# tyb311/TCCT

Measured on AMD Instinct MI355X. Metric: OCT B-scans/sec fwd+bwd(+clip+AdamW), stc_tt bs=8 1x800x1100, higher is better.
Workload: dtype bf16; 1 GPU; stc_tt --los=di bs=8/GPU 1x800x1100 (net tensors 3x800x1104); global_batch=8, parallelism=dp1, ranks=1, grad_allreduce=none, slowest_step=115

## Files before the change

include/tcct_hip.h:

```cpp
#ifndef TCCT_HIP_H
#define TCCT_HIP_H
#include <stdint.h>
#ifdef __cplusplus
extern "C" {
#endif

typedef void* tcct_stream_t;

enum { TCCT_F32 = 0, TCCT_BF16 = 1 };
enum { TCCT_ACT_NONE = 0, TCCT_ACT_LRELU = 1, TCCT_ACT_HSWISH = 2, TCCT_ACT_GELU = 3, TCCT_ACT_SIGMOID = 4,
       TCCT_ACT_ABS = 5 };
enum { TCCT_CRIT_DICE = 0, TCCT_CRIT_DICE2 = 1, TCCT_CRIT_IOU = 2, TCCT_CRIT_MSE = 3 };
enum { TCCT_MCRIT_DICE = 0, TCCT_MCRIT_DICE2 = 1, TCCT_MCRIT_IOU = 2, TCCT_MCRIT_CE = 3 };

int tcct_version(void);
const char* tcct_last_error(void);
int tcct_set_outputs_prezeroed(int on);

int tcct_image_to_nhwc4(const float* img, void* out, int N, int Csrc, int H, int Wsrc, int Wdst, int dtype,
                        tcct_stream_t stream);
int tcct_u8_gather2d(const uint8_t* src, uint8_t* dst, int N, int SH, int SW, int C, int sy0, int sx0, int sh, int sw, int DH, int DW,
                     int dy0, int dx0, int dh, int dw, int flipy, int flipx, int mul, int div, int fill, tcct_stream_t stream);
int tcct_onehot_to_index(const int64_t* onehot, uint8_t* lab, int N, int C, int64_t HW, tcct_stream_t stream);
int tcct_labels_to_u8(const int64_t* lab, uint8_t* out, int N, int H, int Wsrc, int Wdst, tcct_stream_t stream);
// ... 85 lines not shown
                       tcct_stream_t stream);
int tcct_conv32f_pack_weights_sub(const float* w, float* wp, int KH, int KW, int transposed, int cin_total, int o_off, int i_off, tcct_stream_t stream);
int tcct_conv32f_fwd_strided(const float* x, const float* wp, const float* bias, float* y, int N, int H, int W, int KH, int KW, int PH, int PW, int xs,
                             int xo, int ys, int yo, int accumulate, tcct_stream_t stream);
int tcct_conv32f_wgrad_strided(const float* x, const float* dy, float* dw, float* dbias, int N, int H, int W, int KH, int KW, int PH, int PW, int xs,
                               int xo, int ds, int dof, int ldi, int o_off, int i_off, tcct_stream_t stream);
int tcct_pwf_fwd(const float* x, const float* w, const float* bias, float* y, int64_t M, int K, int N, int transposed, tcct_stream_t stream);
int tcct_pwf_wgrad(const float* x, const float* dy, float* dw, float* dbias, int64_t M, int K, int N, tcct_stream_t stream);
int tcct_conv32_pack_weights(const float* w, void* wp, int KH, int KW, int transposed, tcct_stream_t stream);
int tcct_conv32_pack_weights_multi(const void* desc, int n, tcct_stream_t stream);
int tcct_conv32_pack_weights_both(const float* w, void* wp2, int KH, int KW, tcct_stream_t stream);
int tcct_conv32_fwd(const void* x, const void* wp, const float* bias, void* y, int N, int H, int W, int KH, int KW, int PH,
                    int PW, tcct_stream_t stream);

int tcct_conv32_fwd_bnstats(const void* x, const void* wp, const float* bias, void* y, int N, int H, int W, int KH, int KW, int PH,
                            int PW, double* stats, int pre_act, tcct_stream_t stream);
int tcct_conv32_fwd_affine(const void* x, const void* wp, const float* bias, void* y, int N, int H, int W, int KH, int KW,
                           int PH, int PW, const float* ab, int pre_act, int post_act, tcct_stream_t stream);
int tcct_pw_fwd_affine(const void* x, const float* w, const float* bias, void* y, int64_t M, int K, int N, const float* ab,
                       int pre_act, int post_act, int out_dtype, tcct_stream_t stream);
int tcct_pw_fwd_affine_residual(const void* x, const float* w, const float* bias, const float* ab, const void* res, void* y, int64_t M, int K, int N,
                                tcct_stream_t stream);
int tcct_pw_fwd_cat2_affine(const void* x1, const void* x2, const float* w, const float* bias, const float* ab, int post_act, void* y, int64_t M, int K, int N,
                            tcct_stream_t stream);
int tcct_pw_fwd_xaff_affine_residual(const void* y_prev, const float* ab_prev, const float* w, const float* bias, const float* ab, const void* res, void* y,
                                     int64_t M, int K, int N, tcct_stream_t stream);
int tcct_conv32_fwd_add(const void* x, const void* wp, const float* bias, const void* res, void* y, int N, int H, int W, int KH, int KW,
                        int PH, int PW, tcct_stream_t stream);
int tcct_conv32_chain33(const void* x, const void* wp1, const float* bias1, void* mid, const void* wp2, const float* bias2, void* y,
                        const void* res, int N, int H, int W, double* stats, tcct_stream_t stream);
int tcct_conv32_pack_weights_sub(const float* w, void* wp, int KH, int KW, int transposed, int cin_total, int o_off, int i_off,
                                 tcct_stream_t stream);
int tcct_conv32_fwd_strided(const void* x, const void* wp, const float* bias, void* y, int N, int H, int W, int KH, int KW, int PH,
                            int PW, int xs, int xo, int ys, int yo, int accumulate, tcct_stream_t stream);
int tcct_conv32_fwd_strided_bnstats(const void* x, const void* wp, const float* bias, void* y, int N, int H, int W, int KH, int KW, int PH,
                                    int PW, int xs, int xo, int ys, int yo, int accumulate, double* stats, int pre_act, tcct_stream_t stream);
int tcct_conv32_fwd_strided_affine(const void* x, const void* wp, const float* bias, void* y, int N, int H, int W, int KH, int KW, int PH, int PW, int xs,
                                   int xo, int ys, int yo, const float* ab, int pre_act, int post_act, tcct_stream_t stream);
int64_t tcct_conv32_wgrad_mode(int mode);
int64_t tcct_conv32_fwd_mode(int mode);
int tcct_conv32_wgrad_strided(const void* x, const void* dy, float* dw, float* dbias, int N, int H, int W, int KH, int KW, int PH,
                              int PW, int xs, int xo, int ds, int dof, int cin_total, int o_off, int i_off, tcct_stream_t stream);
int tcct_conv32x64_fwd33(const void* x, const void* wp, int wps, const float* bias, void* y, int N, int H, int W, double* stats, int pre_act, int force,
                         tcct_stream_t stream);
int tcct_conv32x64_wgrad33(const void* x, const void* dy, float* dw, float* dbias, int N, int H, int W, int force, tcct_stream_t stream);
int tcct_conv64x32_dgrad33(const void* dy, const void* wp_t, int wps, void* dx, int N, int H, int W, int force, tcct_stream_t stream);
int tcct_conv32_wgrad(const void* x, const void* dy, float* dw, float* dbias, int N, int H, int W, int KH, int KW, int PH,
                      int PW, tcct_stream_t stream);
int tcct_conv32_bwd3x3(const void* x, const void* dy, const void* wp_t, const void* dskip, void* dx, float* dw, float* dbias, int N, int H,
                       int W, tcct_stream_t stream);

int tcct_pw_fwd(const void* x, const float* w, const float* bias, void* y, int64_t M, int K, int N, int transposed,
                int out_dtype, tcct_stream_t stream);
int tcct_pw_wgrad(const void* x, const void* dy, float* dw, float* dbias, int64_t M, int K, int N, tcct_stream_t stream);
int tcct_pw_bwd(const void* x, const void* dy, const float* w, const void* res, void* dx, float* dw, float* dbias, int64_t M, int K, int N,
                tcct_stream_t stream);
int tcct_pw_bwd_cat2(const void* x1, const void* x2, const void* dy, const float* w, void* dx1, void* dx2, float* dw, int64_t M, int K, int N,
                     tcct_stream_t stream);
int tcct_pw_bwd_residual2(const void* x, const void* dy, const float* w, const void* res, void* dx_sum, void* dx_plain, float* dw, float* dbias,
                          int64_t M, int K, int N, tcct_stream_t stream);
int64_t tcct_pw_bwd_bn_supported(int K, int N, int post, int red_post, int split);
int tcct_pw_bwd_bn(const void* x, const void* x2, const void* dz, const void* y, const float* coef, int post, const float* w, const void* res,
                   void* dx, void* dx2, float* dw, float* dbias, int64_t M, int K, int N, const void* y_prev, const float* ab_prev,
                   int red_post, double* sums_prev, tcct_stream_t stream);
int tcct_pw_bwd_bn_sums(const void* x, const void* x2, const void* dz, const void* y, const double* sums, int raw, const float* mean_rstd,
                        const float* ab, float* dgamma, float* dbeta, int post, const float* w, const void* res, void* dx, void* dx2, float* dw,
                        float* dbias, int64_t M, int K, int N, const void* y_prev, const float* ab_prev, int red_post, double* sums_prev,
                        tcct_stream_t stream);
int tcct_pw_wgrad_strided(const void* x, const void* dy, int64_t ldy, float* dw, float* dbias, int64_t M, int K, int N,
                          tcct_stream_t stream);
int tcct_pw_fwd_residual(const void* x, const float* w, const float* bias, const void* res, const float* scale, int64_t per_sample,
                         void* y, void* y_plain, int64_t M, int K, int N, tcct_stream_t stream);
int tcct_pw_fwd_bnstats_xaff(const void* y_prev, const float* ab_prev, const float* w, const float* bias, void* y, int64_t M, int K, int N, double* stats,
                             tcct_stream_t stream);
int tcct_pw_bwd_bn_sums_xaff(const void* y_prev, const float* ab_prev, const void* dz, const void* y, const double* sums, int raw, const float* mean_rstd,
                             const float* ab, float* dgamma, float* dbeta, const float* w, const void* res, void* dx, float* dw, float* dbias, int64_t M,
                             int K, int N, int red_post, double* sums_prev, tcct_stream_t stream);
int tcct_pw_fwd_gelu_residual(const void* x1, const float* w, const float* bias, const void* res, const float* scale, int64_t per_sample, void* y,
                              int64_t M, int K, int N, tcct_stream_t stream);
int tcct_pw_bwd_residual2_sum(const void* x, const void* dy_a, const void* dy_b, const float* w, const void* res, void* dx_sum, void* dx_plain, float* dw,
                              float* dbias, int64_t M, int K, int N, tcct_stream_t stream);
int tcct_pw_bwd_lnb(const void* x, const void* dy, const float* w, const void* t, const float* mean_rstd, const float* gamma, const void* res, void* dt,
                    float* dw, float* dbias, float* dgamma, float* dbeta, int64_t M, int K, int N, tcct_stream_t stream);
int tcct_pw_bwd_gelu(const void* x1, const void* dy, const float* w, void* dx1, float* dw, float* dbias, int64_t M, int K, int N, tcct_stream_t stream);
int tcct_pw_dgrad_residual(const void* dy, const float* w, const void* res, void* dx_sum, void* dx_plain, int64_t M, int Nout, int K,
                           tcct_stream_t stream);
int tcct_pw_fwd_cat2(const void* x1, const void* x2, int K1, const float* w, const float* bias, void* y, int64_t M, int K, int N,
                     double* stats, int pre_act, tcct_stream_t stream);
int tcct_pw_fwd_f32_upadd(const void* x, const float* w, const float* bias, float* y, int B, int uH, int uW, int K, int N, const float* up, tcct_stream_t stream);
int tcct_pw_dgrad_split2(const void* dy, const float* w, void* dx1, void* dx2, int K1, int64_t M, int Nout, int K, tcct_stream_t stream);
int tcct_pw_bwd_cat2_bias(const void* x1, const void* x2, const void* dy, const float* w, void* dx1, void* dx2, float* dw, float* dbias, int64_t M,
                          int K, int N, tcct_stream_t stream);
int tcct_tail_compose(const float* w1, const float* b1, const float* w2, const float* b2, float* wc, float* c, tcct_stream_t stream);
int tcct_tail_compose_bwd(const float* w1, const float* b1, const float* w2, const float* dwc, const float* dc, float* dw1, float* db1, float* dw2,
                          float* db2, tcct_stream_t stream);
int tcct_tail_compose3(const float* w1, const float* b1, const float* w2, const float* b2, const float* w3, const float* b3, int C, float* wcc, float* wa,
                       float* wb, float* ccc, tcct_stream_t stream);
int tcct_tail_compose3_bwd(const float* w1, const float* b1, const float* w2, const float* b2, const float* w3, int C, const float* dwa, const float* dwb,
                           const float* dccc, float* dw1, float* db1, float* dw2, float* db2, float* dw3, float* db3, tcct_stream_t stream);
int tcct_pw_fwd_cat2_f32(const void* x1, const void* x2, int K1, const float* w, const float* bias, float* y, int64_t M, int K, int N, tcct_stream_t stream);
int tcct_head_compose(const float* wt, const float* bt, const float* wa, const float* ba, int C, float* wh, float* ch, tcct_stream_t stream);
int tcct_head_compose_bwd(const float* wt, const float* bt, const float* wa, int C, const float* dwh, const float* dch, float* dwt, float* dbt,
                          float* dwa, float* dba, tcct_stream_t stream);
int tcct_pw_wgrad_cat2(const void* x1, const void* x2, int K1, const void* dy, float* dw, float* dbias, int64_t M, int K, int N,
                       tcct_stream_t stream);
int tcct_pw_fwd_bnstats(const void* x, const float* w, const float* bias, void* y, int64_t M, int K, int N, double* stats, int pre_act,
                        tcct_stream_t stream);

int tcct_im2col3x3_c3(const void* x4, void* out, int N, int H, int W, int stride, int dtype, tcct_stream_t stream);
int tcct_c3_fwd(const void* x4, const float* w, const float* bias, void* y, int B, int H, int W, int stride, double* stats, int stat_pre,
                const float* ab, int pre_act, int post_act, tcct_stream_t stream);
int tcct_c3_wgrad(const void* x4, const void* dy, float* dw, float* dbias, int B, int H, int W, int stride, tcct_stream_t stream);
int tcct_c3_bn_fwd_train(const void* x4, const float* w, const float* bias, void* z, int B, int H, int W, int stride, double* sums,
                         const float* gamma, const float* beta, float eps, float momentum, float* running_mean, float* running_var,
                         int64_t* num_batches_tracked, float* mean_rstd, float* ab, int post_act, tcct_stream_t stream);
int tcct_c3_bn_fwd_eval(const void* x4, const float* w, const float* bias, void* z, int B, int H, int W, int stride, const float* ab, int post_act,
                        tcct_stream_t stream);
int tcct_c3_bn_bwd_reduce(const void* x4, const float* w, const float* bias, const void* dz, int B, int H, int W, int stride, const float* ab,
                          double* raw, int post_act, tcct_stream_t stream);
int tcct_c3_bn_bwd_wgrad(const void* x4, const float* w, const float* bias, const void* dz, int B, int H, int W, int stride, const float* coef,
                         float* dw, float* dbias, int post_act, tcct_stream_t stream);
int64_t tcct_c3_bn_bwd_prefetch(int tiles_ahead);
int tcct_c3_bn_bwd_onepass(const void* x4, const float* w, const float* bias, const void* dz, int B, int H, int W, int stride, const float* mean_rstd,
                           const float* ab, float* work, double* sums, float* dw, float* dbias, float* dgamma, float* dbeta, int post_act, tcct_stream_t stream);
int tcct_pw_wgrad_smalln(const void* x, const void* dy, float* dw, float* dbias, int64_t M, int K, int N, int x_dtype,
                         int dy_dtype, tcct_stream_t stream);

int tcct_stream_copy(const void* src, void* dst, int64_t nbytes, tcct_stream_t stream);

int64_t tcct_kernel_census(int which, int reset);
int tcct_marker(int id, tcct_stream_t stream);

int tcct_dwconv3x3_fwd(const void* x, const float* w, const float* bias, void* y, int N, int H, int W, int C,
                       int stride, int add_input, int dtype, tcct_stream_t stream);
int tcct_dwconv3x3_fwd_bnstats(const void* x, const float* w, const float* bias, void* y, int N, int H, int W, int C, int stride,
                               int add_input, double* stats, int dtype, tcct_stream_t stream);
int tcct_dwconv3x3_dgrad(const void* dy, const float* w, void* dx, int N, int H, int W, int C, int stride,
                         int add_input, int dtype, tcct_stream_t stream);
int tcct_dwconv3x3_dgrad_add(const void* dy, const float* w, const void* res, void* dx, int N, int H, int W, int C, int stride,
                             int add_input, int dtype, tcct_stream_t stream);
int tcct_dwconv3x3_wgrad(const void* x, const void* dy, float* dw, float* dbias, int N, int H, int W, int C,
                         int stride, int dtype, tcct_stream_t stream);
int tcct_dwconv3x3_fwd_xaff(const void* x, const float* xab, const float* w, const float* bias, void* y, int N, int H, int W, int C, int stride,
                            double* stats, int dtype, tcct_stream_t stream);
int tcct_dwconv3x3_wgrad_xaff(const void* x, const float* xab, const void* dy, float* dw, float* dbias, int N, int H, int W, int C, int stride, int dtype,
                              tcct_stream_t stream);
int tcct_dwconv3x3_dgrad_bnred(const void* dy, const float* w, const void* y_prev, const float* ab_prev, void* dx, double* raw, int N, int H, int W, int C,
                               int dtype, tcct_stream_t stream);

int tcct_metapool_fwd(const void* x, void* y, int B, int64_t N, int C, int dtype, tcct_stream_t stream);
int tcct_metapool_bwd(const void* dy, void* dx, int B, int64_t N, int C, int dtype, tcct_stream_t stream);
int tcct_metapool_residual_fwd(const void* x, const void* res, const float* scale, void* y, int B, int64_t N, int C, int dtype,
                               tcct_stream_t stream);
int tcct_metapool_scaled_bwd(const void* dy, const float* scale, void* dx, int B, int64_t N, int C, int dtype, tcct_stream_t stream);
int tcct_ln_metapool_residual_fwd(const void* t, void* y, int B, int64_t N, int C, const float* gamma, const float* beta, float eps, const float* scale,
                                  int dtype, tcct_stream_t stream);
int tcct_ln_metapool_residual_ln_fwd(const void* t, void* y, void* y2, int B, int64_t N, int C, const float* gamma, const float* beta, float eps,
                                     const float* scale, const float* gamma2, const float* beta2, float eps2, float* mean_rstd2, int dtype, tcct_stream_t stream);
int tcct_ln_metapool_residual_bwd(const void* t, const void* dy, void* dt, int B, int64_t N, int C, const float* gamma, float eps, const float* scale,
                                  float* dgamma, float* dbeta, int dtype, tcct_stream_t stream);
int tcct_maxpool2_fwd(const void* x, void* y, int N, int H, int W, int C, int dtype, tcct_stream_t stream);
int tcct_maxpool2_bwd(const void* x, const void* dy, void* dx, int N, int H, int W, int C, int dtype, tcct_stream_t stream);
int tcct_maxpool2_bwd_add(const void* x, const void* dy, const void* res, void* dx, int N, int H, int W, int C, int dtype,
                          tcct_stream_t stream);
int tcct_bilinear_fwd(const void* x, void* y, int N, int H, int W, int C, int Ho, int Wo, int align_corners, int dtype,
                      tcct_stream_t stream);
int tcct_bilinear_bwd_separable(const float* dy, float* dx, float* workspace, int N, int H, int W, int C, int Ho, int Wo,
                                int align_corners, tcct_stream_t stream);
int tcct_bilinear_add_fwd(const void* x, const void* res, void* y, int N, int H, int W, int C, int Ho, int Wo, int align_corners,
                          int dtype, tcct_stream_t stream);
int64_t tcct_bilinear_bwd_x2(int on);
int tcct_bilinear_bwd(const void* dy, void* dx, int N, int H, int W, int C, int Ho, int Wo, int align_corners, int dtype,
                      tcct_stream_t stream);
int tcct_l2norm_fwd(const void* x, void* y, int64_t M, int C, float eps, int dtype, tcct_stream_t stream);
int tcct_l2norm_bwd(const void* x, const void* dy, void* dx, int64_t M, int C, float eps, int dtype, tcct_stream_t stream);
int tcct_l2norm_bwd_scaled(const void* x, const void* dy, void* dx, int64_t M, int C, float eps, float scale, int dtype,
                           tcct_stream_t stream);
int tcct_l2norm_bwd_scaled_add(const void* x, const void* dy, const void* res, void* dx, int64_t M, int C, float eps, float scale, int dtype,
                               tcct_stream_t stream);
int tcct_normadd_fwd(const void* g0, const void* g1, const void* g2, float* inv1, float* inv2, void* out, int N, int H, int W, int C,
                     int h1, int w1, int h2, int w2, float eps, int dtype, tcct_stream_t stream);
int tcct_normadd6_fwd(const void* a0, const void* b0, const void* a1, const void* b1, const void* a2, const void* b2, float* inv1, float* inv2,
                      void* out, int N, int H, int W, int C, int h1, int w1, int h2, int w2, float eps, int dtype, tcct_stream_t stream);
int tcct_l2norm_bwd2_scaled(const void* xa, const void* xb, const void* dn, const void* res_a, const void* res_b, void* da, void* db,
                            int64_t M, int C, float eps, float scale, int dtype, tcct_stream_t stream);

int tcct_softmax_dice_fwd(const void* logits, const uint8_t* labels, int64_t M, int C, double* sums, float* loss,
                          int dtype, tcct_stream_t stream);
int tcct_softmax_dice_bwd(const void* logits, const uint8_t* labels, int64_t M, int C, const double* sums,
                          const float* grad_out, float grad_scale, void* dlogits, int dtype, tcct_stream_t stream);
int tcct_updice_fwd(const float* low, const uint8_t* labels, int B, int h, int w, int H, int W, int C, double* sums, float* loss,
                    tcct_stream_t stream);
int tcct_updice_bwd(const float* low, const uint8_t* labels, int B, int h, int w, int H, int W, int C, const double* sums,
                    const float* grad_out, float grad_scale, float* ws, float* dlow, tcct_stream_t stream);
int tcct_dice_ds_fwd(const void* logits, int dtype, const uint8_t* labels, int B, int H, int W, int C, const float* low1, int h1, int w1, const float* low2,
                     int h2, int w2, const float* low3, int h3, int w3, float coff, double* sums, float* loss, tcct_stream_t stream);
int tcct_softmax_crit_fwd(const void* logits, const uint8_t* labels, int64_t M, int C, int kind, const float* class_w, double* sums, float* loss, int dtype,
                          tcct_stream_t stream);
int tcct_softmax_crit_bwd(const void* logits, const uint8_t* labels, int64_t M, int C, int kind, const float* class_w, const double* sums, const float* grad_out,
                          float grad_scale, void* dlogits, int dtype, tcct_stream_t stream);
int tcct_upcrit_fwd(const float* low, const uint8_t* labels, int B, int h, int w, int H, int W, int C, int kind, const float* class_w, double* sums, float* loss,
                    tcct_stream_t stream);
int tcct_upcrit_bwd(const float* low, const uint8_t* labels, int B, int h, int w, int H, int W, int C, int kind, const float* class_w, const double* sums,
                    const float* grad_out, float grad_scale, float* ws, float* dlow, tcct_stream_t stream);
int tcct_crit_ds_fwd(const void* logits, int dtype, const uint8_t* labels, int B, int H, int W, int C, const float* low1, int h1, int w1, const float* low2, int h2, int w2,
                     const float* low3, int h3, int w3, float coff, int kind, const float* class_w, double* sums, float* loss, tcct_stream_t stream);
int tcct_softmax_mcrit_fwd(const void* logits, const uint8_t* labels, int B, int64_t HW, int C, int kind, const float* class_w, double* sums, float* loss, int dtype,
                           tcct_stream_t stream);
int tcct_softmax_mcrit_bwd(const void* logits, const uint8_t* labels, int B, int64_t HW, int C, int kind, const float* class_w, const double* sums, const float* grad_out,
                           float grad_scale, void* dlogits, int dtype, tcct_stream_t stream);
int tcct_upmcrit_fwd(const float* low, const uint8_t* labels, int B, int h, int w, int H, int W, int C, int kind, const float* class_w, double* sums, float* loss,
                     tcct_stream_t stream);
int tcct_upmcrit_bwd(const float* low, const uint8_t* labels, int B, int h, int w, int H, int W, int C, int kind, const float* class_w, const double* sums,
                     const float* grad_out, float grad_scale, float* ws, float* dlow, tcct_stream_t stream);
int tcct_mcrit_ds_fwd(const void* logits, int dtype, const uint8_t* labels, int B, int H, int W, int C, const float* low1, int h1, int w1, const float* low2, int h2, int w2,
                      const float* low3, int h3, int w3, float coff, int kind, const float* class_w, double* sums, float* loss, tcct_stream_t stream);
int tcct_softmax_pick(const void* logits, const uint8_t* labels, int64_t M, int C, float* prob_lab, uint8_t* argmax,
                      int dtype, tcct_stream_t stream);
int tcct_confusion_counts(const uint8_t* pred, const uint8_t* labels, int N, int64_t HW, int C, float* out,
                          tcct_stream_t stream);

int tcct_gate_fusion_fwd(const void* x1, const void* x2, const float* field, void* y, int N, int H, int W, int C, int hs, int ws,
                         int dtype, tcct_stream_t stream);
int tcct_gate_fusion_bwd(const void* dy, const float* field, void* dx1, void* dx2, int N, int H, int W, int C, int hs, int ws,
                         int dtype, tcct_stream_t stream);

int tcct_mask_boundaries(const uint8_t* mask, int32_t* out, int N, int H, int W, int C, tcct_stream_t stream);

int tcct_slice_channels_fwd(const void* x, float* y, int64_t M, int C, int start, int n, int dtype, tcct_stream_t stream);
int tcct_slice_channels_bwd(const float* dy, void* dx, int64_t M, int C, int start, int n, int dtype, tcct_stream_t stream);
int tcct_label_planes(const uint8_t* labels, float* onehot, float* edge, int N, int H, int W, int start, int n,
                      tcct_stream_t stream);
int tcct_gumbel_colsoftmax_fwd(const float* x, const float* eps, float* out, float* stats, int N, int H, int W, int CH,
                               tcct_stream_t stream);
int tcct_gumbel_colsoftmax_bwd(const float* x, const float* eps, const float* stats, const float* dout, float* dx, int N,
                               int H, int W, int CH, tcct_stream_t stream);
int tcct_colsoftmax_fwd(const float* x, float* y, int N, int H, int W, tcct_stream_t stream);
int tcct_colsoftmax_bwd(const float* y, const float* dy, float* dx, int N, int H, int W, tcct_stream_t stream);
int tcct_colwsum_fwd(const float* x, const float* wts, float* out, int N, int H, int W, tcct_stream_t stream);
int tcct_colwsum_bwd(const float* dout, const float* wts, float* dx, int N, int H, int W, tcct_stream_t stream);
int tcct_mse_fwd(const float* a, const float* b, int64_t n, double* acc, float* out, tcct_stream_t stream);
// ... 55 lines not shown
```

tcct_amd/__init__.py:

```python
__version__ = '0.1.0'

import os as _os
import warnings as _warnings

RETIRED_ENV = frozenset('''TCCT_BILINEAR_VEC8 TCCT_BN_DEFER TCCT_BN_DEFER_DW TCCT_BN_FUSE TCCT_BN_POOL TCCT_BN_RED TCCT_BN_RED_DW TCCT_BN_VEC8 TCCT_C3_BN TCCT_C3_DIRECT
TCCT_C3_ONEPASS TCCT_CONV_STREAM TCCT_DP_MARKS TCCT_DS_DICE TCCT_DW_CPT TCCT_DW_WGRAD_CPT TCCT_DW_WGRAD_SIDE TCCT_DY2 TCCT_F32_MFMA TCCT_FPL_LAZY_GRAD
TCCT_FUSED_CONV_BWD TCCT_FUSED_PW_BWD TCCT_FUSE_AUX TCCT_GRAPH_ERRMODE TCCT_GRAPH_SHARED_POOL TCCT_HEAD_COMPOSE TCCT_HEAD_UPADD TCCT_LN_POOL TCCT_LN_POOL_LN2
TCCT_MLP_GELU TCCT_MLP_TAIL TCCT_NORMADD_BAND TCCT_PACK_ALL TCCT_PW_FWD2 TCCT_TAIL_AUX TCCT_TAIL_AUX_LOW TCCT_TAIL_COMPOSE TCCT_TRAN_FUSE TCCT_TRAN_RED2
TCCT_WGRAD_FRESH_EVENT TCCT_WGRAD_GENERIC TCCT_WGRAD_LINE TCCT_WGRAD_RECORD_STREAM TCCT_WGRAD_STREAM'''.split())
_set = sorted(v for v in RETIRED_ENV if v in _os.environ)
if _set:
    _warnings.warn('tcct_amd: ' + ', '.join(_set) + ' no longer have any effect (retired environment switches; use the tcct_amd.ops module constants or '
                   '`bench.py --set NAME=0|1`)', RuntimeWarning, stacklevel=2)
```

tcct_amd/csrc/common.h:

```cpp
#pragma once
#include <hip/hip_runtime.h>
#include <hip/hip_bf16.h>
#include <stdint.h>
#include <stdio.h>
#include "../../include/tcct_hip.h"

typedef __hip_bfloat16 bf16;

void tcct_set_error(const char* fmt, ...);
enum { TCCT_CENSUS_CHAIN33 = 0, TCCT_CENSUS_WGRADK_STREAM = 1, TCCT_CENSUS_WGRAD33_STREAM = 2, TCCT_CENSUS_FWD33_STREAM = 3, TCCT_CENSUS_N = 8 };
void tcct_census_hit(int which);
int tcct_skip_zero_fill();

#define TCCT_CHECK(cond, ...)                                   \
    do {                                                        \
        if (!(cond)) {                                          \
            tcct_set_error(__VA_ARGS__);                        \
            return -1;                                          \
        }                                                       \
    } while (0)

#define TCCT_LAUNCH_OK()                                                        \
    do {                                                                        \
        hipError_t e__ = hipGetLastError();                                     \
// ... 77 lines not shown
    const uint4 t = *reinterpret_cast<const uint4*>(p);
    const uint32_t w[4] = {t.x, t.y, t.z, t.w};
#pragma unroll
    for (int j = 0; j < 4; ++j) { o[2 * j] = __uint_as_float(w[j] << 16); o[2 * j + 1] = __uint_as_float(w[j] & 0xffff0000u); }
}
template <int VEC> __device__ __forceinline__ void stv(float* p, const float* v) {
    if (VEC == 1) { *p = v[0]; return; }
#pragma unroll
    for (int j = 0; j < VEC / 4; ++j) *reinterpret_cast<float4*>(p + 4 * j) = make_float4(v[4 * j], v[4 * j + 1], v[4 * j + 2], v[4 * j + 3]);
}
template <int VEC> __device__ __forceinline__ void stv(bf16* p, const float* v) {
    if (VEC == 1) { *p = __float2bfloat16(v[0]); return; }
    if (VEC == 4) { uint2 t; t.x = pack_bf16x2(v[0], v[1]); t.y = pack_bf16x2(v[2], v[3]); *reinterpret_cast<uint2*>(p) = t; return; }
    uint4 t;
    t.x = pack_bf16x2(v[0], v[1]); t.y = pack_bf16x2(v[2], v[3]); t.z = pack_bf16x2(v[4], v[5]); t.w = pack_bf16x2(v[6], v[7]);
    *reinterpret_cast<uint4*>(p) = t;
}

__device__ __forceinline__ float erf_fast(float x) {
    const float ax = fabsf(x);
    const float t = __builtin_amdgcn_rcpf(1.f + 0.3275911f * ax);
    const float poly = t * (0.254829592f + t * (-0.284496736f + t * (1.421413741f + t * (-1.453152027f + t * 1.061405429f))));
    const float r = 1.f - poly * __expf(-ax * ax);
    return copysignf(r, x);
}
__device__ __forceinline__ void gauss_cdf_pdf(float x, float& cdf, float& pdf) {
    const float e = __expf(-0.5f * x * x);
    const float t = __builtin_amdgcn_rcpf(1.f + 0.23164189f * fabsf(x));
    const float poly = t * (0.254829592f + t * (-0.284496736f + t * (1.421413741f + t * (-1.453152027f + t * 1.061405429f))));
    const float h = 0.5f * poly * e;
    cdf = x >= 0.f ? 1.f - h : h;
    pdf = 0.3989422804014327f * e;
}
__device__ __forceinline__ float act_fwd(int kind, float x) {
    switch (kind) {
        case TCCT_ACT_LRELU: return x > 0.f ? x : 0.01f * x;
        case TCCT_ACT_HSWISH: return x * fminf(fmaxf(x + 3.f, 0.f), 6.f) * (1.f / 6.f);
        case TCCT_ACT_GELU: { float c, p; gauss_cdf_pdf(x, c, p); return x * c; }
        case TCCT_ACT_SIGMOID: return 1.f / (1.f + __expf(-x));
        case TCCT_ACT_ABS: return fabsf(x);
        default: return x;
    }
}
__device__ __forceinline__ float act_grad(int kind, float x) {
    switch (kind) {
        case TCCT_ACT_LRELU: return x > 0.f ? 1.f : 0.01f;
        case TCCT_ACT_HSWISH: return x < -3.f ? 0.f : (x <= 3.f ? (2.f * x + 3.f) * (1.f / 6.f) : 1.f);
        case TCCT_ACT_GELU: { float c, p; gauss_cdf_pdf(x, c, p); return c + x * p; }
        case TCCT_ACT_SIGMOID: { float s = 1.f / (1.f + __expf(-x)); return s * (1.f - s); }
        case TCCT_ACT_ABS: return x > 0.f ? 1.f : (x < 0.f ? -1.f : 0.f);
        default: return 1.f;
    }
}

template <int KIND> __device__ __forceinline__ float act_c(float x) {
    if (KIND == TCCT_ACT_LRELU) return x > 0.f ? x : 0.01f * x;
    if (KIND == TCCT_ACT_HSWISH) return x * fminf(fmaxf(x + 3.f, 0.f), 6.f) * (1.f / 6.f);
    if (KIND == TCCT_ACT_GELU) { float c, p; gauss_cdf_pdf(x, c, p); return x * c; }
    if (KIND == TCCT_ACT_SIGMOID) return 1.f / (1.f + __expf(-x));
    if (KIND == TCCT_ACT_ABS) return fabsf(x);
    return x;
}
template <int PRE, int POST> __device__ __forceinline__ void affine4_c(float* v, const float* a, const float* b) {
#pragma unroll
    for (int i = 0; i < 4; ++i) v[i] = act_c<POST>(a[i] * act_c<PRE>(v[i]) + b[i]);
}
__device__ __forceinline__ void affine4(float* v, const float* a, const float* b, int pre, int post) {
    if (pre == TCCT_ACT_NONE && post == TCCT_ACT_NONE) affine4_c<TCCT_ACT_NONE, TCCT_ACT_NONE>(v, a, b);
    else if (pre == TCCT_ACT_NONE && post == TCCT_ACT_HSWISH) affine4_c<TCCT_ACT_NONE, TCCT_ACT_HSWISH>(v, a, b);
    else if (pre == TCCT_ACT_NONE && post == TCCT_ACT_LRELU) affine4_c<TCCT_ACT_NONE, TCCT_ACT_LRELU>(v, a, b);
    else if (pre == TCCT_ACT_LRELU && post == TCCT_ACT_NONE) affine4_c<TCCT_ACT_LRELU, TCCT_ACT_NONE>(v, a, b);
    else if (pre == TCCT_ACT_NONE && post == TCCT_ACT_GELU) affine4_c<TCCT_ACT_NONE, TCCT_ACT_GELU>(v, a, b);
    else {
#pragma unroll
        for (int i = 0; i < 4; ++i) v[i] = act_fwd(post, a[i] * act_fwd(pre, v[i]) + b[i]);
    }
}

__device__ __forceinline__ void wave_lds_fence() {
    __builtin_amdgcn_fence(__ATOMIC_ACQ_REL, "wavefront");
}

typedef __attribute__((__vector_size__(4 * sizeof(unsigned int)))) unsigned int u32x4;
__device__ __forceinline__ void lds_dma16(const u32x4& rsrc, uint32_t voff, uint32_t lds_addr) {
    unsigned keep;
    asm volatile("s_nop 4\n\ts_mov_b32 %0, m0\n\ts_mov_b32 m0, %3\n\ts_nop 0\n\tbuffer_load_dwordx4 %1, %2, 0 offen lds\n\ts_mov_b32 m0, %0"
                 : "=&s"(keep) : "v"(voff), "s"(rsrc), "s"(lds_addr) : "memory");
}
__device__ __forceinline__ u32x4 make_rsrc_words(const void* base, uint32_t bytes) {
    const uint64_t b = (uint64_t)base;
    u32x4 d;
    d[0] = __builtin_amdgcn_readfirstlane((uint32_t)b);
    d[1] = __builtin_amdgcn_readfirstlane((uint32_t)(b >> 32) & 0xffffu);
    d[2] = __builtin_amdgcn_readfirstlane(bytes);
    d[3] = 0x00020000u;
    return d;
}

template <typename T> __device__ __forceinline__ float round_as(float v);
template <> __device__ __forceinline__ float round_as<float>(float v) { return v; }
template <> __device__ __forceinline__ float round_as<bf16>(float v) { return __bfloat162float(__float2bfloat16(v)); }

__device__ __forceinline__ unsigned xcd_band(unsigned b, unsigned n) {
    const unsigned q = n >> 3, r = n & 7u, x = b & 7u, k = b >> 3;
    return x * q + (x < r ? x : r) + k;
}

struct Lerp { int i0, i1; float l0, l1; };
__device__ __forceinline__ Lerp src_index(int o, float scale, int in, int align) {
    float s = align ? scale * (float)o : fmaxf(scale * ((float)o + 0.5f) - 0.5f, 0.f);
    Lerp r;
    r.i0 = min((int)s, in - 1);
    r.i1 = r.i0 + (r.i0 < in - 1 ? 1 : 0);
    r.l1 = s - (float)r.i0;
    r.l0 = 1.f - r.l1;
    return r;
}

__device__ __forceinline__ float row16_sum(float v) {
    v += __builtin_bit_cast(float, __builtin_amdgcn_update_dpp(0, __builtin_bit_cast(int, v), 0xB1, 0xF, 0xF, true));
    v += __builtin_bit_cast(float, __builtin_amdgcn_update_dpp(0, __builtin_bit_cast(int, v), 0x4E, 0xF, 0xF, true));
    v += __builtin_bit_cast(float, __builtin_amdgcn_update_dpp(0, __builtin_bit_cast(int, v), 0x141, 0xF, 0xF, true));
    v += __builtin_bit_cast(float, __builtin_amdgcn_update_dpp(0, __builtin_bit_cast(int, v), 0x140, 0xF, 0xF, true));
    return v;
}
__device__ __forceinline__ float lane_group_sum(float v, int LP) {
    if (LP >= 2) v += __builtin_bit_cast(float, __builtin_amdgcn_update_dpp(0, __builtin_bit_cast(int, v), 0xB1, 0xF, 0xF, true));
    if (LP >= 4) v += __builtin_bit_cast(float, __builtin_amdgcn_update_dpp(0, __builtin_bit_cast(int, v), 0x4E, 0xF, 0xF, true));
    if (LP >= 8) v += __builtin_bit_cast(float, __builtin_amdgcn_update_dpp(0, __builtin_bit_cast(int, v), 0x141, 0xF, 0xF, true));
    if (LP >= 16) v += __builtin_bit_cast(float, __builtin_amdgcn_update_dpp(0, __builtin_bit_cast(int, v), 0x140, 0xF, 0xF, true));
    for (int o = 16; o < LP; o <<= 1) v += __shfl_xor(v, o, 64);
    return v;
}
__device__ __forceinline__ float wave_sum(float v) {
#pragma unroll
    for (int o = 32; o > 0; o >>= 1) v += __shfl_xor(v, o, 64);
    return v;
}
__device__ __forceinline__ float wave_max(float v) {
#pragma unroll
    for (int o = 32; o > 0; o >>= 1) v = fmaxf(v, __shfl_xor(v, o, 64));
    return v;
}
__device__ __forceinline__ float block_sum(float v, float* sm ) {
    v = wave_sum(v);
    int w = threadIdx.x >> 6, nw = blockDim.x >> 6;
    __syncthreads();
    if ((threadIdx.x & 63) == 0) sm[w] = v;
    __syncthreads();
    float r = 0.f;
    for (int i = 0; i < nw; ++i) r += sm[i];
    return r;
}
```

tcct_amd/csrc/ln_pool.hip:

```cpp
#include "common.h"

#define LP_T 256

struct f8 { float v[8]; };
__device__ __forceinline__ f8 ld8(const float* p) {
    const float4 a = *reinterpret_cast<const float4*>(p), b = *reinterpret_cast<const float4*>(p + 4);
    return f8{{a.x, a.y, a.z, a.w, b.x, b.y, b.z, b.w}};
}
__device__ __forceinline__ f8 ld8(const bf16* p) {
    const uint4 t = *reinterpret_cast<const uint4*>(p);
    return f8{{__uint_as_float(t.x << 16), __uint_as_float(t.x & 0xffff0000u), __uint_as_float(t.y << 16), __uint_as_float(t.y & 0xffff0000u),
               __uint_as_float(t.z << 16), __uint_as_float(t.z & 0xffff0000u), __uint_as_float(t.w << 16), __uint_as_float(t.w & 0xffff0000u)}};
}
__device__ __forceinline__ void st8(float* p, const f8& a) {
    *reinterpret_cast<float4*>(p) = make_float4(a.v[0], a.v[1], a.v[2], a.v[3]);
    *reinterpret_cast<float4*>(p + 4) = make_float4(a.v[4], a.v[5], a.v[6], a.v[7]);
}
__device__ __forceinline__ void st8(bf16* p, const f8& a) {
    uint4 t;
    t.x = pack_bf16x2(a.v[0], a.v[1]); t.y = pack_bf16x2(a.v[2], a.v[3]); t.z = pack_bf16x2(a.v[4], a.v[5]); t.w = pack_bf16x2(a.v[6], a.v[7]);
    *reinterpret_cast<uint4*>(p) = t;
}
__device__ __forceinline__ f8 f8zero() { return f8{{0.f, 0.f, 0.f, 0.f, 0.f, 0.f, 0.f, 0.f}}; }

struct Row10 { float g[10]; };
template <int LP>
__device__ __forceinline__ Row10 widen(const f8& m, bool hasl, bool hasr) {
    Row10 o;
    const float ls = __shfl_up(m.v[7], 1, LP), rs = __shfl_down(m.v[0], 1, LP);
    o.g[0] = hasl ? ls : 0.f;
#pragma unroll
    for (int k = 0; k < 8; ++k) o.g[1 + k] = m.v[k];
    o.g[9] = hasr ? rs : 0.f;
    return o;
}

template <typename T> struct Raw8;
template <> struct Raw8<bf16> { uint4 v; };
template <> struct Raw8<float> { float4 a, b; };
__device__ __forceinline__ Raw8<bf16> ldraw(const bf16* p) { return Raw8<bf16>{*reinterpret_cast<const uint4*>(p)}; }
__device__ __forceinline__ Raw8<float> ldraw(const float* p) { return Raw8<float>{*reinterpret_cast<const float4*>(p), *reinterpret_cast<const float4*>(p + 4)}; }
__device__ __forceinline__ f8 unpack(const Raw8<bf16>& r) {
    const uint4 t = r.v;
    return f8{{__uint_as_float(t.x << 16), __uint_as_float(t.x & 0xffff0000u), __uint_as_float(t.y << 16), __uint_as_float(t.y & 0xffff0000u),
               __uint_as_float(t.z << 16), __uint_as_float(t.z & 0xffff0000u), __uint_as_float(t.w << 16), __uint_as_float(t.w & 0xffff0000u)}};
}
__device__ __forceinline__ f8 unpack(const Raw8<float>& r) { return f8{{r.a.x, r.a.y, r.a.z, r.a.w, r.b.x, r.b.y, r.b.z, r.b.w}}; }
template <typename T> __device__ __forceinline__ Raw8<T> raw_zero();
template <> __device__ __forceinline__ Raw8<bf16> raw_zero<bf16>() { return Raw8<bf16>{make_uint4(0u, 0u, 0u, 0u)}; }
template <> __device__ __forceinline__ Raw8<float> raw_zero<float>() { return Raw8<float>{make_float4(0.f, 0.f, 0.f, 0.f), make_float4(0.f, 0.f, 0.f, 0.f)}; }

#define LNP_STRIP 32
#define LNP_PF 4
#ifndef LNP_PF_FWD
#define LNP_PF_FWD 4
#endif

template <int LP>
__device__ __forceinline__ void row_stats(const f8& x, bool act, float invC, float eps, float& mean, float& rstd) {
    float s = 0.f;
#pragma unroll
    for (int k = 0; k < 8; ++k) s += x.v[k];
    s = lane_group_sum(s, LP);
    mean = s * invC;
    float q = 0.f;
#pragma unroll
    for (int k = 0; k < 8; ++k) { const float d = act ? x.v[k] - mean : 0.f; q += d * d; }
    q = lane_group_sum(q, LP);
    rstd = rsqrtf(q * invC + eps);
}

template <typename T, int LP, bool LN2>
__global__ void __launch_bounds__(LP_T)
k_ln_metapool_fwd(const T* __restrict__ t, T* __restrict__ y, int N, int C, const float* __restrict__ gamma, const float* __restrict__ beta, float eps,
                  const float* __restrict__ scale, T* __restrict__ y2, const float* __restrict__ gamma2, const float* __restrict__ beta2, float eps2,
                  float* __restrict__ mean_rstd2) {
    constexpr int GPB = LP_T / LP, S = LNP_STRIP, PF = LNP_PF_FWD;
    const int gl = threadIdx.x % LP, grp = threadIdx.x / LP;
    const int c0 = gl * 8;
    const bool act = c0 < C;
    const bool hasl = act && c0 > 0, hasr = act && c0 + 8 < C;
    float gam[8], bet[8], cs[8];
#pragma unroll
    for (int k = 0; k < 8; ++k) {
        gam[k] = act ? gamma[c0 + k] : 0.f; bet[k] = act ? beta[c0 + k] : 0.f;
        const int c = c0 + k;
        cs[k] = 1.f / (float)(1 + (c > 0) + (c < C - 1));
    }
    float gam2[8], bet2[8];
#pragma unroll
    for (int k = 0; k < 8; ++k) { gam2[k] = (LN2 && act) ? gamma2[c0 + k] : 0.f; bet2[k] = (LN2 && act) ? beta2[c0 + k] : 0.f; }
    const int64_t img = (int64_t)blockIdx.y * N;
    const T* tb = t + img * C + c0;
    T* yb = y + img * C + c0;
    const float sc = scale ? scale[blockIdx.y] : 1.f;
    const float invC = 1.f / (float)C;
    const int n0 = (blockIdx.x * GPB + grp) * S;
    if (n0 >= N) return;
    auto fetch = [&](int nn) { return (act && nn >= 0 && nn < N) ? ldraw(tb + (int64_t)nn * C) : raw_zero<T>(); };
    auto normed = [&](const f8& x, int nn, f8& ctr) {
        float mean, rstd;
        row_stats<LP>(x, act, invC, eps, mean, rstd);
        const bool in = nn >= 0 && nn < N;
#pragma unroll
        for (int k = 0; k < 8; ++k) ctr.v[k] = (in && act) ? round_as<T>((x.v[k] - mean) * rstd * gam[k] + bet[k]) : 0.f;
        return widen<LP>(ctr, hasl, hasr);
    };
    const Raw8<T> r0 = fetch(n0 - 1), r1 = fetch(n0);
    Raw8<T> ring[PF];
#pragma unroll
    for (int j = 0; j < PF; ++j) ring[j] = fetch(n0 + 1 + j);
    f8 cprev, ccur, cnxt;
    f8 e = unpack(r1);
    Row10 prev = normed(unpack(r0), n0 - 1, cprev), cur = normed(e, n0, ccur);
    for (int i0 = 0; i0 < S; i0 += PF) {
#pragma unroll
        for (int j = 0; j < PF; ++j) {
            const int n = n0 + i0 + j;
            const f8 xn = unpack(ring[j]);
            ring[j] = fetch(n + 1 + PF);
            const Row10 nxt = normed(xn, n + 1, cnxt);
            if (n < N) {
                const float rinv = 1.f / (float)(1 + (n > 0) + (n < N - 1));
                f8 o;
#pragma unroll
                for (int k = 0; k < 8; ++k) {
                    float s_ = (prev.g[k] + cur.g[k] + nxt.g[k]) + (prev.g[k + 1] + cur.g[k + 1] + nxt.g[k + 1]) + (prev.g[k + 2] + cur.g[k + 2] + nxt.g[k + 2]);
                    s_ *= rinv * cs[k];
                    o.v[k] = e.v[k] + sc * (s_ - ccur.v[k]);
                }
                if (act) st8(yb + (int64_t)n * C, o);
                if (LN2) {
                    f8 orr;
#pragma unroll
                    for (int k = 0; k < 8; ++k) orr.v[k] = act ? round_as<T>(o.v[k]) : 0.f;
                    float mean2, rstd2;
                    row_stats<LP>(orr, act, invC, eps2, mean2, rstd2);
                    if (gl == 0) { mean_rstd2[2 * (img + n)] = mean2; mean_rstd2[2 * (img + n) + 1] = rstd2; }
                    f8 b;
#pragma unroll
                    for (int k = 0; k < 8; ++k) b.v[k] = (orr.v[k] - mean2) * rstd2 * gam2[k] + bet2[k];
                    if (act) st8(y2 + (img + n) * C + c0, b);
                }
            }
            prev = cur; cur = nxt; ccur = cnxt; e = xn;
        }
    }
}

template <typename T, int LP>
__global__ void __launch_bounds__(LP_T, sizeof(T) == 2 ? 3 : 2)
k_ln_metapool_bwd(const T* __restrict__ t, const T* __restrict__ dy, T* __restrict__ dt, int N, int C, const float* __restrict__ gamma, float eps,
                  const float* __restrict__ scale, float* __restrict__ dgamma, float* __restrict__ dbeta) {
    constexpr int GPB = LP_T / LP, S = LNP_STRIP, PF = LNP_PF;
    __shared__ float swv[(LP_T / 64) * 2 * 8 * LP];
    const int gl = threadIdx.x % LP, grp = threadIdx.x / LP;
    const int c0 = gl * 8;
    const bool act = c0 < C;
    const bool hasl = act && c0 > 0, hasr = act && c0 + 8 < C;
    float gam[8], cs[10];
#pragma unroll
    for (int k = 0; k < 8; ++k) gam[k] = act ? gamma[c0 + k] : 0.f;
#pragma unroll
    for (int j = 0; j < 10; ++j) {
        const int c = c0 - 1 + j;
        cs[j] = 1.f / (float)(1 + (c > 0) + (c < C - 1));
    }
    const int64_t img = (int64_t)blockIdx.y * N;
    const T* tb = t + img * C + c0;
    const T* db = dy + img * C + c0;
    T* ob = dt + img * C + c0;
    const float sc = scale ? scale[blockIdx.y] : 1.f;
    const float invC = 1.f / (float)C;
    const int n0 = (blockIdx.x * GPB + grp) * S;
    float ag[8], ab[8];
#pragma unroll
    for (int k = 0; k < 8; ++k) { ag[k] = 0.f; ab[k] = 0.f; }
    auto fetchd = [&](int nn) { return (act && nn >= 0 && nn < N) ? ldraw(db + (int64_t)nn * C) : raw_zero<T>(); };
    auto fetchx = [&](int nn) { return (act && nn >= 0 && nn < N) ? ldraw(tb + (int64_t)nn * C) : raw_zero<T>(); };
    auto weighted = [&](const f8& d, int nn) {
        Row10 o = widen<LP>(d, hasl, hasr);
        const float rw = 1.f / (float)(1 + (nn > 0) + (nn < N - 1));
#pragma unroll
        for (int j = 0; j < 10; ++j) o.g[j] *= rw * cs[j];
        return o;
    };
    if (n0 < N) {
        const Raw8<T> q0 = fetchd(n0 - 1), q1 = fetchd(n0);
        Raw8<T> dring[PF], xring[PF];
#pragma unroll
        for (int j = 0; j < PF; ++j) { dring[j] = fetchd(n0 + 1 + j); xring[j] = fetchx(n0 + j); }
        f8 dcur = unpack(q1);
        Row10 prev = weighted(unpack(q0), n0 - 1), cur = weighted(dcur, n0);
        for (int i0 = 0; i0 < S; i0 += PF) {
#pragma unroll
            for (int j = 0; j < PF; ++j) {
                const int n = n0 + i0 + j;
                const f8 dn = unpack(dring[j]);
                dring[j] = fetchd(n + 1 + PF);
                const f8 xc = unpack(xring[j]);
                xring[j] = fetchx(n + PF);
                const Row10 nxt = weighted(dn, n + 1);
                float mean, rstd;
                row_stats<LP>(xc, act, invC, eps, mean, rstd);
                if (n < N) {
                    float g[8], xh[8], s1 = 0.f, s2 = 0.f;
#pragma unroll
                    for (int k = 0; k < 8; ++k) {
                        const float s_ = (prev.g[k] + cur.g[k] + nxt.g[k]) + (prev.g[k + 1] + cur.g[k + 1] + nxt.g[k + 1]) + (prev.g[k + 2] + cur.g[k + 2] + nxt.g[k + 2]);
                        const float da = act ? round_as<T>(sc * (s_ - dcur.v[k])) : 0.f;
                        const float h = act ? (xc.v[k] - mean) * rstd : 0.f;
                        xh[k] = h;
                        ag[k] += da * h;
                        ab[k] += da;
                        g[k] = da * gam[k];
                        s1 += g[k]; s2 += g[k] * h;
                    }
                    s1 = lane_group_sum(s1, LP) * invC; s2 = lane_group_sum(s2, LP) * invC;
                    f8 o;
#pragma unroll
                    for (int k = 0; k < 8; ++k) o.v[k] = rstd * (g[k] - s1 - xh[k] * s2) + dcur.v[k];
                    if (act) st8(ob + (int64_t)n * C, o);
                }
                prev = cur; cur = nxt; dcur = dn;
            }
        }
    }
    const int wv = threadIdx.x >> 6, lane = threadIdx.x & 63;
#pragma unroll
    for (int k = 0; k < 8; ++k) {
        float a = ag[k], b = ab[k];
        for (int o = LP; o < 64; o <<= 1) { a += __shfl_xor(a, o, 64); b += __shfl_xor(b, o, 64); }
        if (lane < LP) { swv[(wv * 2 + 0) * 8 * LP + c0 + k] = a; swv[(wv * 2 + 1) * 8 * LP + c0 + k] = b; }
    }
    __syncthreads();
    for (int c = threadIdx.x; c < C; c += LP_T) {
        float a = 0.f, b = 0.f;
#pragma unroll
        for (int w2 = 0; w2 < LP_T / 64; ++w2) { a += swv[(w2 * 2 + 0) * 8 * LP + c]; b += swv[(w2 * 2 + 1) * 8 * LP + c]; }
        atomicAdd(&dgamma[c], a); atomicAdd(&dbeta[c], b);
    }
}

static bool ln_metapool_shape_ok(int B, int64_t N, int C) { return C % 8 == 0 && C >= 16 && C <= 256 && B >= 1 && B <= 65535 && N >= 1 && N < (1LL << 30); }
static int ln_metapool_fwd_impl(const void* t, void* y, int B, int64_t N, int C, const float* gamma, const float* beta, float eps, const float* scale, void* y2,
                                const float* gamma2, const float* beta2, float eps2, float* mean_rstd2, int dtype, tcct_stream_t stream) {
    TCCT_CHECK(ln_metapool_shape_ok(B, N, C), "ln_metapool_residual_fwd: B=%d N=%lld C=%d unsupported (C %% 8 == 0, 16 <= C <= 256)", B, (long long)N, C);
    TCCT_CHECK(t && y && gamma && beta, "ln_metapool_residual_fwd: NULL argument");
    const int64_t strips = (N + LNP_STRIP - 1) / LNP_STRIP;
#define LNPF(LP_, L2) hipLaunchKernelGGL((k_ln_metapool_fwd<T, LP_, L2>), dim3((unsigned)((strips + LP_T / LP_ - 1) / (LP_T / LP_)), (unsigned)B), dim3(LP_T), 0, \
                                         (hipStream_t)stream, (const T*)t, (T*)y, (int)N, C, gamma, beta, eps, scale, (T*)y2, gamma2, beta2, eps2, mean_rstd2)
    if (y2) { TCCT_DISPATCH(dtype, if (C <= 64) LNPF(8, true); else if (C <= 128) LNPF(16, true); else LNPF(32, true)); }
    else { TCCT_DISPATCH(dtype, if (C <= 64) LNPF(8, false); else if (C <= 128) LNPF(16, false); else LNPF(32, false)); }
#undef LNPF
    TCCT_LAUNCH_OK();
}
extern "C" int tcct_ln_metapool_residual_fwd(const void* t, void* y, int B, int64_t N, int C, const float* gamma, const float* beta, float eps, const float* scale,
                                             int dtype, tcct_stream_t stream) {
    return ln_metapool_fwd_impl(t, y, B, N, C, gamma, beta, eps, scale, nullptr, nullptr, nullptr, 0.f, nullptr, dtype, stream);
}
extern "C" int tcct_ln_metapool_residual_ln_fwd(const void* t, void* y, void* y2, int B, int64_t N, int C, const float* gamma, const float* beta, float eps,
                                                const float* scale, const float* gamma2, const float* beta2, float eps2, float* mean_rstd2, int dtype,
                                                tcct_stream_t stream) {
    TCCT_CHECK(y2 && gamma2 && beta2 && mean_rstd2, "ln_metapool_residual_ln_fwd: NULL argument");
    return ln_metapool_fwd_impl(t, y, B, N, C, gamma, beta, eps, scale, y2, gamma2, beta2, eps2, mean_rstd2, dtype, stream);
}
extern "C" int tcct_ln_metapool_residual_bwd(const void* t, const void* dy, void* dt, int B, int64_t N, int C, const float* gamma, float eps, const float* scale,
                                             float* dgamma, float* dbeta, int dtype, tcct_stream_t stream) {
    TCCT_CHECK(ln_metapool_shape_ok(B, N, C), "ln_metapool_residual_bwd: B=%d N=%lld C=%d unsupported (C %% 8 == 0, 16 <= C <= 256)", B, (long long)N, C);
    TCCT_CHECK(t && dy && dt && gamma && dgamma && dbeta, "ln_metapool_residual_bwd: NULL argument");
    hipStream_t st = (hipStream_t)stream;
    if (!tcct_skip_zero_fill() && (hipMemsetAsync(dgamma, 0, sizeof(float) * C, st) != hipSuccess || hipMemsetAsync(dbeta, 0, sizeof(float) * C, st) != hipSuccess)) {
        tcct_set_error("ln_metapool_residual_bwd: memset failed"); return -2;
    }
    const int64_t strips = (N + LNP_STRIP - 1) / LNP_STRIP;
#define LNPB(LP_) hipLaunchKernelGGL((k_ln_metapool_bwd<T, LP_>), dim3((unsigned)((strips + LP_T / LP_ - 1) / (LP_T / LP_)), (unsigned)B), dim3(LP_T), 0, st, (const T*)t, \
                                     (const T*)dy, (T*)dt, (int)N, C, gamma, eps, scale, dgamma, dbeta)
    TCCT_DISPATCH(dtype, if (C <= 64) LNPB(8); else if (C <= 128) LNPB(16); else LNPB(32));
#undef LNPB
    TCCT_LAUNCH_OK();
}
```

tcct_amd/csrc/pw_mfma.hip:

```cpp
#include "common.h"
#include "c3_geom.h"
#include <cstdlib>

typedef __attribute__((ext_vector_type(8))) __bf16 bf16x8;
typedef __attribute__((ext_vector_type(16))) float f32x16;
typedef __attribute__((ext_vector_type(4))) short s16x4;
typedef __attribute__((ext_vector_type(8))) short s16x8;

#define PWB 256

__device__ __forceinline__ void st_out4(bf16* p, float a, float b, float c, float d) {
    uint2 o; o.x = pack_bf16x2(a, b); o.y = pack_bf16x2(c, d);
    *reinterpret_cast<uint2*>(p) = o;
}
__device__ __forceinline__ void st_out4(float* p, float a, float b, float c, float d) {
    *reinterpret_cast<float4*>(p) = make_float4(a, b, c, d);
}


struct PwUp { const float* p; int uH, uW, Ho, Wo; float sh, sw; uint32_t m_howo, m_wo; };
struct PwSplit { const bf16* x2; int K1; void* y2; int N1; const bf16* res; const float* rscale; int64_t per_sample; bf16* yplain; C3Geom c3; PwUp up; };
template <int NT, typename Tout, bool STATS, bool AFF, bool C3 = false>
__global__ void __launch_bounds__(PWB, 2)
k_pw_fwd(const bf16* __restrict__ x, const float* __restrict__ w, const float* __restrict__ bias, Tout* __restrict__ y,
// ... 606 lines not shown
        else
        if (co < N && ci_base + cl < K) atomicAdd(&dw[(int64_t)co * K + ci_base + cl], red[i]);
    }
    if (dbias && blockIdx.y == 0) {
#pragma unroll
        for (int ct = 0; ct < NT; ++ct) {
            float s = bsum[ct] + __shfl_xor(bsum[ct], 32, 64);
            if (lane < 32 && ct * 32 + r < N) atomicAdd(&dbias[ct * 32 + r], s);
        }
    }
}

static int pw_wgrad_impl(const void* x, const void* x2, int K1, const void* dy, float* dw, float* dbias, int64_t M, int K, int N, tcct_stream_t stream,
                         int64_t ldy);
extern "C" int tcct_pw_wgrad(const void* x, const void* dy, float* dw, float* dbias, int64_t M, int K, int N, tcct_stream_t stream) {
    return pw_wgrad_impl(x, nullptr, 0, dy, dw, dbias, M, K, N, stream, 0);
}
extern "C" int tcct_pw_wgrad_cat2(const void* x1, const void* x2, int K1, const void* dy, float* dw, float* dbias, int64_t M, int K, int N,
                                  tcct_stream_t stream) {
    TCCT_CHECK(x2 != nullptr && K1 % 32 == 0 && K1 > 0 && K1 < K, "pw_wgrad_cat2: K1=%d must be a multiple of 32 inside (0, K)", K1);
    return pw_wgrad_impl(x1, x2, K1, dy, dw, dbias, M, K, N, stream, 0);
}
extern "C" int tcct_pw_wgrad_strided(const void* x, const void* dy, int64_t ldy, float* dw, float* dbias, int64_t M, int K, int N,
                                     tcct_stream_t stream) {
    return pw_wgrad_impl(x, nullptr, 0, dy, dw, dbias, M, K, N, stream, ldy);
}
static int pw_wgrad_impl(const void* x, const void* x2, int K1, const void* dy, float* dw, float* dbias, int64_t M, int K, int N, tcct_stream_t stream,
                         int64_t ldy) {
    if (ldy == 0) ldy = N;
    TCCT_CHECK(ldy >= N && ldy % 8 == 0, "pw_wgrad: ldy=%lld must be a multiple of 8 and >= N=%d", (long long)ldy, N);
    TCCT_CHECK(K % 32 == 0 && N % 32 == 0 && K >= 32 && N >= 32 && N <= 160 && K <= 1024, "pw_wgrad: unsupported K=%d N=%d", K, N);
    hipStream_t st = (hipStream_t)stream;
    if (!tcct_skip_zero_fill() && hipMemsetAsync(dw, 0, sizeof(float) * (size_t)N * K, st) != hipSuccess) { tcct_set_error("pw_wgrad: memset failed"); return -2; }
    if (dbias && !tcct_skip_zero_fill() && hipMemsetAsync(dbias, 0, sizeof(float) * N, st) != hipSuccess) { tcct_set_error("pw_wgrad: memset failed"); return -2; }
    const int NT = N / 32, ktiles = K / 32;
    const int KTB = (ktiles % 2 == 0 && NT <= 2) ? 2 : 1;
    const int gy = ktiles / KTB;
    TCCT_CHECK(!x2 || K1 % (KTB * 32) == 0, "pw_wgrad_cat2: K1=%d must be a multiple of %d for this shape", K1, KTB * 32);
    const int SX = KTB == 1 ? 64 : 192;
    const int SD = 2 * N + ((NT & 1) ? 0 : 64);
    size_t lds = (size_t)PW_P * (SX + SD);
    size_t red = (size_t)NT * 32 * KTB * 32 * 4;
    if (red > lds) lds = red;
    const int64_t tiles = (M + PW_P - 1) / PW_P;
    int per_cu = (int)((160 * 1024) / (lds + 512));
    if (per_cu > 2) per_cu = 2;
    if (per_cu < 1) per_cu = 1;
    int gx = 256 * per_cu / gy;
    if (gx < 64) gx = 64;
    if (tiles <= 1024) { int small = 128 / gy; if (small < 16) small = 16; if (gx > small) gx = small; }
    if (gx > tiles) gx = (int)tiles;
    if (gx < 1) gx = 1;
#define WL(NTV, KV) tcct_launch<k_pw_wgrad<NTV, KV>, 160 * 1024>(dim3(gx, gy), dim3(PWB), lds, st, (const bf16*)x, (const bf16*)dy, dw, dbias, M, K, N, SX, SD, (const bf16*)x2, K1, ldy, C3Geom{})
    if (KTB == 2) { switch (NT) { case 1: WL(1, 2); break; default: WL(2, 2); break; } }
    else { switch (NT) { case 1: WL(1, 1); break; case 2: WL(2, 1); break; case 3: WL(3, 1); break; case 4: WL(4, 1); break; default: WL(5, 1); break; } }
#undef WL
    TCCT_LAUNCH_OK();
}


extern "C" int tcct_c3_wgrad(const void* x4, const void* dy, float* dw, float* dbias, int B, int H, int W, int stride, tcct_stream_t stream) {
    TCCT_CHECK(stride == 1 || stride == 2, "c3_wgrad: stride %d", stride);
    const int Ho = (H - 1) / stride + 1, Wo = (W - 1) / stride + 1;
    const int64_t M = (int64_t)B * Ho * Wo, inb = (int64_t)B * H * W * 8;
    TCCT_CHECK(M > 0 && M * 64 < (1ll << 31) && inb < (1ll << 31), "c3_wgrad: image too large for 32-bit byte offsets (B=%d H=%d W=%d)", B, H, W);
    hipStream_t st = (hipStream_t)stream;
    if (!tcct_skip_zero_fill() && hipMemsetAsync(dw, 0, sizeof(float) * 32 * 27, st) != hipSuccess) { tcct_set_error("c3_wgrad: memset failed"); return -2; }
    if (dbias && !tcct_skip_zero_fill() && hipMemsetAsync(dbias, 0, sizeof(float) * 32, st) != hipSuccess) { tcct_set_error("c3_wgrad: memset failed"); return -2; }
    const int SX = 192, SD = 64;
    const size_t lds = (size_t)PW_P * (SX + SD);
    const int64_t tiles = (M + PW_P - 1) / PW_P;
    int gx = (int)(tiles / 48 < 256 ? 256 : (tiles / 48 > 1024 ? 1024 : tiles / 48));
    if (gx > tiles) gx = (int)tiles;
    auto magic = [](uint32_t d) { return d == 1 ? 0xffffffffu : (uint32_t)((1ull << 32) / d); };
    hipLaunchKernelGGL((k_pw_wgrad<1, 2, true>), dim3(gx, 1), dim3(PWB), lds, st, (const bf16*)x4, (const bf16*)dy, dw, dbias, M, 64, 32, SX, SD,
                       (const bf16*)nullptr, 0, (int64_t)32,
                       C3Geom{H, W, Ho, Wo, stride, (uint32_t)inb, (Wo + 31) / 32, magic((uint32_t)((Wo + 31) / 32)), magic((uint32_t)Ho), magic((uint32_t)(Ho * Wo)), magic((uint32_t)Wo)});
    TCCT_LAUNCH_OK();
}


#define PB_P 128

__device__ __forceinline__ u32x4 gelu8(u32x4 v) {
    u32x4 o;
#pragma unroll
    for (int k = 0; k < 4; ++k)
        o[k] = pack_bf16x2(act_c<TCCT_ACT_GELU>(__uint_as_float(v[k] << 16)), act_c<TCCT_ACT_GELU>(__uint_as_float(v[k] & 0xffff0000u)));
    return o;
}
__device__ __forceinline__ float gelu_grad1(float x) { float c, p; gauss_cdf_pdf(x, c, p); return c + x * p; }
template <int KIND> __device__ __forceinline__ u32x4 affine8(u32x4 v, const float* __restrict__ a, const float* __restrict__ b) {
    const float4 a0 = *reinterpret_cast<const float4*>(a), a1 = *reinterpret_cast<const float4*>(a + 4);
    const float4 b0 = *reinterpret_cast<const float4*>(b), b1 = *reinterpret_cast<const float4*>(b + 4);
    const float aa[8] = {a0.x, a0.y, a0.z, a0.w, a1.x, a1.y, a1.z, a1.w}, bb[8] = {b0.x, b0.y, b0.z, b0.w, b1.x, b1.y, b1.z, b1.w};
    u32x4 o;
#pragma unroll
    for (int k = 0; k < 4; ++k)
        o[k] = pack_bf16x2(act_c<KIND>(aa[2 * k] * __uint_as_float(v[k] << 16) + bb[2 * k]),
                           act_c<KIND>(aa[2 * k + 1] * __uint_as_float(v[k] & 0xffff0000u) + bb[2 * k + 1]));
    return o;
}
struct PwBnBwd { const bf16* y; const float* coef; const bf16* yprev; const float* abprev; double* sums_prev;
                 const double* sums; int raw; const float* mean_rstd; const float* ab; float* dgamma; float* dbeta; };
template <int KIND> __device__ __forceinline__ float pw_act_grad(float u) {
    if (KIND == TCCT_ACT_HSWISH) return u < -3.f ? 0.f : (u <= 3.f ? (2.f * u + 3.f) * (1.f / 6.f) : 1.f);
    return 1.f;
}
template <int NT, int KT, bool SPLIT = false, int BNP = -1, int REDP = -1, bool GX = false, int XAP = -1, bool LNB = false, bool DY2 = false>
__global__ void __launch_bounds__(PWB, 2)
k_pw_bwd(const bf16* __restrict__ x, const bf16* __restrict__ dy, const float* __restrict__ w, const bf16* __restrict__ res,
         bf16* __restrict__ dx, bf16* __restrict__ dx_plain, float* __restrict__ dw, float* __restrict__ dbias, int64_t M, PwBnBwd bn) {
    constexpr int K = 32 * KT, N = 32 * NT;
    constexpr bool BN = BNP >= 0, RED = REDP >= 0;
    constexpr int SX = 64 * KT + ((KT & 1) ? 0 : 64), SD = 64 * NT + ((NT & 1) ? 0 : 64);
    constexpr int SW = 2 * N + 16;
    constexpr int XS = K / 16, DS = N / 16;
    extern __shared__ __attribute__((aligned(16))) unsigned char smem[];
    unsigned char* sX = smem;
    unsigned char* sD = sX + PB_P * SX;
    unsigned char* sW = sD + PB_P * SD;
    unsigned char* sS = sW + ((K * SW + 15) & ~15);
    float* sC = reinterpret_cast<float*>(sS + 4 * 2560);
    float* sP = sC + (BN ? 5 * N : 0);
    const int tid = threadIdx.x, lane = tid & 63, wave = tid >> 6;
    const int r = lane & 31, hh = lane >> 5;
    for (int i = tid; i < N * K; i += PWB) {
        const int n = i / K, k = i - n * K;
        *reinterpret_cast<bf16*>(sW + k * SW + n * 2) = __float2bfloat16(w[i]);
    }
    if (BN) {
        if (bn.coef) { for (int i = tid; i < 5 * N; i += PWB) sC[i] = bn.coef[i]; }
        else if (tid < N) {
            const int c = tid;
            const double mu = bn.mean_rstd[c], rs = bn.mean_rstd[N + c];
            const double S1 = bn.sums[c];
            const double S2 = bn.raw ? (bn.sums[N + c] - mu * S1) * rs : bn.sums[N + c];
            if (blockIdx.x == 0) { bn.dbeta[c] = (float)S1; bn.dgamma[c] = (float)S2; }
            const double a = bn.ab[c], s1 = S1 / (double)M, s2 = S2 / (double)M;
            sC[c] = (float)a; sC[N + c] = (float)(-a * s2 * rs); sC[2 * N + c] = (float)(a * (s2 * rs * mu - s1));
            sC[3 * N + c] = bn.ab[c]; sC[4 * N + c] = bn.ab[N + c];
        }
    }
    if (RED || XAP >= 0) for (int i = tid; i < 2 * (SPLIT ? K / 2 : K); i += PWB) sP[i] = bn.abprev[i];
    if (LNB) for (int i = tid; i < K; i += PWB) sP[i] = bn.abprev[i];
    constexpr int RKT = LNB ? KT : (RED ? (SPLIT ? KT / 2 : KT) : 1);
    float rs[RKT][8], rq[RKT][8];
#pragma unroll
    for (int a = 0; a < RKT; ++a)
#pragma unroll
        for (int k = 0; k < 8; ++k) rs[a][k] = rq[a][k] = 0.f;
    f32x16 accw[(NT * KT + 3) / 4];
#pragma unroll
    for (int a = 0; a < (NT * KT + 3) / 4; ++a)
#pragma unroll
        for (int k = 0; k < 16; ++k) accw[a][k] = 0.f;
    float bsum[(NT * KT + 3) / 4];
#pragma unroll
    for (int a = 0; a < (NT * KT + 3) / 4; ++a) bsum[a] = 0.f;
    const int64_t tiles = (M + PB_P - 1) / PB_P;
    constexpr int KS = SPLIT ? K / 2 : K;
    const uint32_t xbytes = (uint32_t)(M * KS * 2), dbytes = (uint32_t)(M * N * 2);
    const __amdgpu_buffer_rsrc_t rx = __builtin_amdgcn_make_buffer_rsrc((void*)x, 0, xbytes, 0x00020000);
    const __amdgpu_buffer_rsrc_t rd = __builtin_amdgcn_make_buffer_rsrc((void*)dy, 0, dbytes, 0x00020000);
    const __amdgpu_buffer_rsrc_t rr = __builtin_amdgcn_make_buffer_rsrc((void*)(res ? res : x), 0, xbytes, 0x00020000);
    const __amdgpu_buffer_rsrc_t ro = __builtin_amdgcn_make_buffer_rsrc((void*)dx, 0, xbytes, 0x00020000);
    const __amdgpu_buffer_rsrc_t rp = __builtin_amdgcn_make_buffer_rsrc((void*)(dx_plain ? dx_plain : dx), 0, xbytes, 0x00020000);
    const __amdgpu_buffer_rsrc_t ry = __builtin_amdgcn_make_buffer_rsrc((void*)((BN || DY2) ? bn.y : dy), 0, dbytes, 0x00020000);
    const __amdgpu_buffer_rsrc_t ryp = __builtin_amdgcn_make_buffer_rsrc((void*)((RED || LNB) ? bn.yprev : x), 0, xbytes, 0x00020000);
    u32x4 px[XS], pd[DS], py[(BN || DY2) ? DS : 1];
    auto prefetch = [&](int64_t tile) {
        const uint32_t bx = (uint32_t)(tile * PB_P * KS * 2), bd = (uint32_t)(tile * PB_P * N * 2);
#pragma unroll
        for (int j = 0; j < XS; ++j) {
            if (SPLIT && j >= XS / 2) px[j] = __builtin_amdgcn_raw_buffer_load_b128(rr, bx + (uint32_t)(tid + (j - XS / 2) * PWB) * 16u, 0, 0);
            else px[j] = __builtin_amdgcn_raw_buffer_load_b128(rx, bx + (uint32_t)(tid + j * PWB) * 16u, 0, 0);
        }
#pragma unroll
        for (int j = 0; j < DS; ++j) pd[j] = __builtin_amdgcn_raw_buffer_load_b128(rd, bd + (uint32_t)(tid + j * PWB) * 16u, 0, 0);
        if (BN || DY2) {
#pragma unroll
            for (int j = 0; j < DS; ++j) py[j] = __builtin_amdgcn_raw_buffer_load_b128(ry, bd + (uint32_t)(tid + j * PWB) * 16u, 0, 0);
        }
    };
    auto stage_x1 = [&](int j, u32x4 xv_) {
        const int jj = (SPLIT && j >= XS / 2) ? j - XS / 2 : j;
        const int q = tid + jj * PWB, p = q / (KS / 8), c = q - p * (KS / 8);
        if (GX) xv_ = gelu8(xv_);
        if (XAP >= 0) xv_ = affine8<XAP < 0 ? 0 : XAP>(xv_, sP + c * 8, sP + KS + c * 8);
        *reinterpret_cast<u32x4*>(sX + p * SX + ((SPLIT && j >= XS / 2) ? KS * 2 : 0) + c * 16) = xv_;
    };
    auto stage_d = [&](int64_t tile) {
#pragma unroll
        for (int j = 0; j < DS; ++j) {
            const int q = tid + j * PWB, p = q / (N / 8), c = q - p * (N / 8);
            u32x4 v = pd[j];
            if (DY2) {
#pragma unroll
                for (int k = 0; k < 4; ++k)
                    v[k] = pack_bf16x2(__uint_as_float(pd[j][k] << 16) + __uint_as_float(py[j][k] << 16),
                                       __uint_as_float(pd[j][k] & 0xffff0000u) + __uint_as_float(py[j][k] & 0xffff0000u));
            }
            if (BN) {
                const bool live = tile * PB_P + p < M;
                const float* cc = sC + c * 8;
#pragma unroll
                for (int h = 0; h < 2; ++h) {
                    const float4 c1 = *reinterpret_cast<const float4*>(cc + 4 * h), c2 = *reinterpret_cast<const float4*>(cc + N + 4 * h);
                    const float4 c3 = *reinterpret_cast<const float4*>(cc + 2 * N + 4 * h);
                    float4 ca = c1, cb = c1;
                    if (BNP != TCCT_ACT_NONE) { ca = *reinterpret_cast<const float4*>(cc + 3 * N + 4 * h); cb = *reinterpret_cast<const float4*>(cc + 4 * N + 4 * h); }
                    const float k1[4] = {c1.x, c1.y, c1.z, c1.w}, k2[4] = {c2.x, c2.y, c2.z, c2.w}, k3[4] = {c3.x, c3.y, c3.z, c3.w};
                    const float ka[4] = {ca.x, ca.y, ca.z, ca.w}, kb[4] = {cb.x, cb.y, cb.z, cb.w};
#pragma unroll
                    for (int e2 = 0; e2 < 2; ++e2) {
                        const uint32_t gz = pd[j][2 * h + e2], gy = py[j][2 * h + e2];
                        float z0 = __uint_as_float(gz << 16), z1 = __uint_as_float(gz & 0xffff0000u);
                        const float y0 = __uint_as_float(gy << 16), y1 = __uint_as_float(gy & 0xffff0000u);
                        if (BNP != TCCT_ACT_NONE) {
                            z0 *= pw_act_grad<BNP>(ka[2 * e2] * y0 + kb[2 * e2]);
                            z1 *= pw_act_grad<BNP>(ka[2 * e2 + 1] * y1 + kb[2 * e2 + 1]);
                        }
                        const float o0 = k1[2 * e2] * z0 + k2[2 * e2] * y0 + k3[2 * e2];
                        const float o1 = k1[2 * e2 + 1] * z1 + k2[2 * e2 + 1] * y1 + k3[2 * e2 + 1];
                        v[2 * h + e2] = live ? pack_bf16x2(o0, o1) : 0u;
                    }
                }
            }
            *reinterpret_cast<u32x4*>(sD + p * SD + c * 16) = v;
        }
    };
    auto stage = [&](int64_t tile) {
#pragma unroll
        for (int j = 0; j < XS; ++j) stage_x1(j, px[j]);
        stage_d(tile);
    };
    const int li = lane & 15, lq = li >> 2, lpp = li & 3, lg = lane >> 4;
    const int lrow = 8 * (lg >> 1) + lq, lcol = (16 * (lg & 1) + 4 * lpp) * 2;
    const unsigned char* lbX = sX + lrow * SX + lcol;
    const unsigned char* lbD = sD + lrow * SD + lcol;
    auto tr2 = [&](const unsigned char* p, int stride) {
        s16x4 lo = __builtin_amdgcn_ds_read_tr16_b64_v4i16((__attribute__((address_space(3))) s16x4*)p);
        s16x4 hi = __builtin_amdgcn_ds_read_tr16_b64_v4i16((__attribute__((address_space(3))) s16x4*)(p + 4 * stride));
        s16x8 v = __builtin_shufflevector(lo, hi, 0, 1, 2, 3, 4, 5, 6, 7);
        return __builtin_bit_cast(bf16x8, v);
    };
    int64_t tile = blockIdx.x;
    if (tile < tiles) {
        prefetch(tile);
        __syncthreads();
        stage(tile);
        prefetch(tile + gridDim.x);
    }
    __syncthreads();
    for (; tile < tiles; tile += gridDim.x) {
        u32x4 xq[GX ? KT : 1][2];
        if (GX) {
            const int64_t m0q = tile * PB_P + 32 * wave;
#pragma unroll
            for (int kt = 0; kt < KT; ++kt)
#pragma unroll
                for (int h2 = 0; h2 < 2; ++h2) {
                    const int64_t mm = m0q + (lane >> 2) + 16 * h2;
                    xq[kt][h2] = __builtin_amdgcn_raw_buffer_load_b128(rx, mm < M ? (uint32_t)((mm * K + kt * 32 + (lane & 3) * 8) * 2) : 0x80000000u, 0, 0);
                }
        }
        u32x4 tq[LNB ? KT : 1][2];
        float tmean[2] = {0.f, 0.f}, trstd[2] = {0.f, 0.f};
        if (LNB) {
            const int64_t m0q = tile * PB_P + 32 * wave;
#pragma unroll
// ... 171 lines not shown
                    if (dx_plain) __builtin_amdgcn_raw_buffer_store_b128(o, rp, off, 0, 0);
                    const u32x4 rv = __builtin_amdgcn_raw_buffer_load_b128(rr, off, 0, 0);
#pragma unroll
                    for (int k = 0; k < 4; ++k)
                        o[k] = pack_bf16x2(__uint_as_float(o[k] << 16) + __uint_as_float(rv[k] << 16),
                                           __uint_as_float(o[k] & 0xffff0000u) + __uint_as_float(rv[k] & 0xffff0000u));
                }
                __builtin_amdgcn_raw_buffer_store_b128(o, ro, off, 0, 0);
                if (RED) red_acc(o, kt * 32 + cch * 8);
            }
            wave_lds_fence();
        }
        __syncthreads();
    }
    if (RED) {
        __syncthreads();
        float* red = reinterpret_cast<float*>(smem);
        constexpr int KR = SPLIT ? K / 2 : K;
#pragma unroll
        for (int kt = 0; kt < RKT; ++kt) {
#pragma unroll
            for (int k = 0; k < 8; ++k) {
                float a = rs[kt][k], b = rq[kt][k];
#pragma unroll
                for (int o = 32; o > 2; o >>= 1) { a += __shfl_xor(a, o, 64); b += __shfl_xor(b, o, 64); }
                if (lane < 4) {
                    red[wave * 2 * KR + kt * 32 + 8 * lane + k] = a;
                    red[wave * 2 * KR + KR + kt * 32 + 8 * lane + k] = b;
                }
            }
        }
        __syncthreads();
        for (int i2 = tid; i2 < KR; i2 += PWB) {
            double a = 0.0, b = 0.0;
#pragma unroll
            for (int wv = 0; wv < 4; ++wv) { a += (double)red[wv * 2 * KR + i2]; b += (double)red[wv * 2 * KR + KR + i2]; }
            atomicAdd(&bn.sums_prev[i2], a); atomicAdd(&bn.sums_prev[KR + i2], b);
        }
        __syncthreads();
    }
    if (LNB) {
        __syncthreads();
        float* red = reinterpret_cast<float*>(smem);
#pragma unroll
        for (int kt = 0; kt < KT; ++kt) {
#pragma unroll
            for (int k = 0; k < 8; ++k) {
                float a = rs[kt][k], b = rq[kt][k];
#pragma unroll
                for (int o = 32; o > 2; o >>= 1) { a += __shfl_xor(a, o, 64); b += __shfl_xor(b, o, 64); }
                if (lane < 4) {
                    red[wave * 2 * K + kt * 32 + 8 * lane + k] = a;
                    red[wave * 2 * K + K + kt * 32 + 8 * lane + k] = b;
                }
            }
        }
        __syncthreads();
        for (int i2 = tid; i2 < K; i2 += PWB) {
            float a = 0.f, b = 0.f;
#pragma unroll
            for (int wv = 0; wv < 4; ++wv) { a += red[wv * 2 * K + i2]; b += red[wv * 2 * K + K + i2]; }
            atomicAdd(&bn.dgamma[i2], a); atomicAdd(&bn.dbeta[i2], b);
        }
        __syncthreads();
    }
#pragma unroll
    for (int a = 0; a < (NT * KT + 3) / 4; ++a) {
        const int ti = wave + 4 * a;
        if (ti < NT * KT) {
            const int ct = ti / KT, kt = ti - ct * KT;
#pragma unroll
            for (int k = 0; k < 16; ++k) {
                const int co = ct * 32 + (k & 3) + 8 * (k >> 2) + 4 * hh;
                atomicAdd(&dw[(int64_t)co * K + kt * 32 + r], accw[a][k]);
            }
            if (dbias && kt == 0) {
                const float sb = bsum[a] + __shfl_xor(bsum[a], 32, 64);
                if (lane < 32) atomicAdd(&dbias[ct * 32 + r], sb);
            }
        }
    }
}

struct PwBwdMode { bool split = false; int bnp = -1, redp = -1; bool gelu_x = false; int xap = -1; bool lnb = false, dy2 = false; };
static PwBnBwd pw_bn_coef(const void* y, const float* coef, const void* y_prev, const float* ab_prev, double* sums_prev) {
    PwBnBwd b{};
    b.y = (const bf16*)y; b.coef = coef; b.yprev = (const bf16*)y_prev; b.abprev = ab_prev; b.sums_prev = sums_prev;
    return b;
}
static PwBnBwd pw_bn_sums(const void* y, const double* sums, int raw, const float* mean_rstd, const float* ab, float* dgamma, float* dbeta, const void* y_prev,
                          const float* ab_prev, double* sums_prev) {
    PwBnBwd b = pw_bn_coef(y, nullptr, y_prev, ab_prev, sums_prev);
    b.sums = sums; b.raw = raw; b.mean_rstd = mean_rstd; b.ab = ab; b.dgamma = dgamma; b.dbeta = dbeta;
    return b;
}
static PwBnBwd pw_bn_ln_front(const void* t, const float* gamma, const float* mean_rstd, float* dgamma, float* dbeta) {
    PwBnBwd b{};
    b.yprev = (const bf16*)t; b.abprev = gamma; b.mean_rstd = mean_rstd; b.dgamma = dgamma; b.dbeta = dbeta;
    return b;
}
static PwBnBwd pw_bn_dy2(const void* dy_b) {
    PwBnBwd b{};
    b.y = (const bf16*)dy_b;
    return b;
}

typedef void (*PwBwdLaunch)(dim3, dim3, size_t, hipStream_t, const bf16*, const bf16*, const float*, const bf16*, bf16*, bf16*, float*, float*, int64_t, PwBnBwd);
struct PwBwdRow { int nt, kt; bool split; int bnp, redp; bool gx; int xap; bool lnb, dy2; PwBwdLaunch launch; };
static_assert(TCCT_ACT_HSWISH == 2 && TCCT_ACT_NONE == 0, "activation codes are template arguments below");
#define PWB_ROW(NT, KT, SP, BN, RD, GX, XA, LN, D2) {NT, KT, SP, BN, RD, GX, XA, LN, D2, tcct_launch<k_pw_bwd<NT, KT, SP, BN, RD, GX, XA, LN, D2>, 160 * 1024>}
#define PWB_PLAIN(NT, KT, SP) PWB_ROW(NT, KT, SP, -1, -1, false, -1, false, false)
#define PWB_BN(NT, KT, SP, BN, RD) PWB_ROW(NT, KT, SP, BN, RD, false, -1, false, false)
static const PwBwdRow pw_bwd_table[] = {
    PWB_PLAIN(1, 1, false), PWB_PLAIN(1, 2, false), PWB_PLAIN(1, 3, false), PWB_PLAIN(1, 4, false),
    PWB_PLAIN(2, 1, false), PWB_PLAIN(2, 2, false), PWB_PLAIN(2, 3, false), PWB_PLAIN(2, 4, false),
    PWB_PLAIN(3, 1, false), PWB_PLAIN(3, 2, false), PWB_PLAIN(3, 3, false), PWB_PLAIN(3, 4, false),
    PWB_PLAIN(4, 1, false), PWB_PLAIN(4, 2, false), PWB_PLAIN(4, 3, false), PWB_PLAIN(4, 4, false),
    PWB_PLAIN(1, 4, true), PWB_PLAIN(2, 4, true), PWB_PLAIN(3, 4, true), PWB_PLAIN(4, 4, true), PWB_PLAIN(1, 2, true),
    PWB_BN(1, 1, false, 0, -1), PWB_BN(1, 3, false, 0, -1), PWB_BN(1, 4, false, 0, -1),
    PWB_BN(2, 2, false, 0, -1), PWB_BN(2, 2, false, 2, -1), PWB_BN(3, 3, false, 0, -1), PWB_BN(3, 3, false, 2, -1), PWB_BN(3, 4, true, 2, -1),
    PWB_BN(2, 2, false, 0, 0), PWB_BN(2, 2, false, 0, 2), PWB_BN(2, 2, false, 2, 0), PWB_BN(2, 2, false, 2, 2),
    PWB_ROW(2, 2, false, 0, 2, false, 2, false, false), PWB_ROW(3, 3, false, 0, -1, false, 2, false, false),
    PWB_ROW(2, 2, false, -1, -1, true, -1, false, false), PWB_ROW(3, 3, false, -1, -1, true, -1, false, false),
    PWB_ROW(2, 2, false, -1, -1, false, -1, true, false),
    PWB_ROW(1, 1, false, -1, -1, false, -1, false, true),
};
#undef PWB_BN
#undef PWB_PLAIN
#undef PWB_ROW
static const PwBwdRow* pw_bwd_find(int K, int N, const PwBwdMode& md) {
    if (K % 32 || N % 32) return nullptr;
    for (const PwBwdRow& r : pw_bwd_table)
        if (r.nt == N / 32 && r.kt == K / 32 && r.split == md.split && r.bnp == md.bnp && r.redp == md.redp && r.gx == md.gelu_x && r.xap == md.xap && r.lnb == md.lnb &&
            r.dy2 == md.dy2) return &r;
    return nullptr;
}

static int pw_bwd_impl(const void* x, const void* dy, const float* w, const void* res, void* dx, void* dx_plain, float* dw, float* dbias,
                       int64_t M, int K, int N, tcct_stream_t stream, const PwBwdMode& md = PwBwdMode(), PwBnBwd bn = PwBnBwd{}) {
    const PwBwdRow* row = pw_bwd_find(K, N, md);
    TCCT_CHECK(row != nullptr, "pw_bwd: K=%d N=%d unsupported: no kernel for NT=%d KT=%d SPLIT=%d BNP=%d REDP=%d GX=%d XAP=%d LNB=%d DY2=%d", K, N, N / 32, K / 32,
               (int)md.split, md.bnp, md.redp, (int)md.gelu_x, md.xap, (int)md.lnb, (int)md.dy2);
    TCCT_CHECK(M > 0 && M * (int64_t)(K > N ? K : N) * 2 < (1LL << 31), "pw_bwd: tensor exceeds the 2 GiB buffer-descriptor range");
    const int NT = N / 32, KT = K / 32;
    const int SX = 64 * KT + ((KT & 1) ? 0 : 64), SD = 64 * NT + ((NT & 1) ? 0 : 64), SW = 2 * N + 16;
    const size_t lds = (size_t)PB_P * (SX + SD) + (((size_t)K * SW + 15) & ~(size_t)15) + 4 * 2560 + (md.bnp >= 0 ? (size_t)5 * N * 4 : 0) +
                       ((md.redp >= 0 || md.xap >= 0 || md.lnb) ? (size_t)2 * K * 4 : 0);
    TCCT_CHECK(lds <= 160 * 1024, "pw_bwd: %zu B of LDS", lds);
    hipStream_t st = (hipStream_t)stream;
    if (!tcct_skip_zero_fill()) {
        bool ok = true;
        if (md.redp >= 0) ok = ok && hipMemsetAsync(bn.sums_prev, 0, sizeof(double) * 2 * (md.split ? K / 2 : K), st) == hipSuccess;
        if (md.lnb) ok = ok && hipMemsetAsync(bn.dgamma, 0, sizeof(float) * K, st) == hipSuccess && hipMemsetAsync(bn.dbeta, 0, sizeof(float) * K, st) == hipSuccess;
        ok = ok && hipMemsetAsync(dw, 0, sizeof(float) * (size_t)N * K, st) == hipSuccess;
        if (dbias) ok = ok && hipMemsetAsync(dbias, 0, sizeof(float) * N, st) == hipSuccess;
        if (!ok) { tcct_set_error("pw_bwd: memset failed"); return -2; }
    }
    const int64_t tiles = (M + PB_P - 1) / PB_P;
    int per_cu = (int)((160 * 1024) / (lds + 256));
    if (per_cu > 2) per_cu = 2;
    int64_t gx = 256 * per_cu;
    if (gx > tiles) gx = tiles;
    row->launch(dim3((unsigned)gx), dim3(PWB), lds, st, (const bf16*)x, (const bf16*)dy, w, (const bf16*)res, (bf16*)dx, (bf16*)dx_plain, dw, dbias, M, bn);
    TCCT_LAUNCH_OK();
}
static PwBwdMode pw_bwd_split() { PwBwdMode md; md.split = true; return md; }
extern "C" int tcct_pw_bwd_cat2(const void* x1, const void* x2, const void* dy, const float* w, void* dx1, void* dx2, float* dw, int64_t M,
                                int K, int N, tcct_stream_t stream) {
    TCCT_CHECK(K == 128 && x2 != nullptr && dx2 != nullptr, "pw_bwd_cat2: two halves of 64 channels only (K=%d)", K);
    return pw_bwd_impl(x1, dy, w, x2, dx1, dx2, dw, nullptr, M, K, N, stream, pw_bwd_split());
}
extern "C" int tcct_pw_bwd_cat2_bias(const void* x1, const void* x2, const void* dy, const float* w, void* dx1, void* dx2, float* dw, float* dbias,
                                     int64_t M, int K, int N, tcct_stream_t stream) {
    TCCT_CHECK(x2 != nullptr && dx2 != nullptr, "pw_bwd_cat2_bias: x2 or dx2 is NULL (K=%d N=%d: 128 -> any, or 64 -> 32)", K, N);
    return pw_bwd_impl(x1, dy, w, x2, dx1, dx2, dw, dbias, M, K, N, stream, pw_bwd_split());
}
extern "C" int tcct_pw_bwd(const void* x, const void* dy, const float* w, const void* res, void* dx, float* dw, float* dbias, int64_t M,
                           int K, int N, tcct_stream_t stream) {
    return pw_bwd_impl(x, dy, w, res, dx, nullptr, dw, dbias, M, K, N, stream);
}
extern "C" int tcct_pw_bwd_residual2(const void* x, const void* dy, const float* w, const void* res, void* dx_sum, void* dx_plain, float* dw,
                                     float* dbias, int64_t M, int K, int N, tcct_stream_t stream) {
    TCCT_CHECK(res != nullptr && dx_plain != nullptr && dx_plain != dx_sum, "pw_bwd_residual2: needs res and two distinct outputs");
    return pw_bwd_impl(x, dy, w, res, dx_sum, dx_plain, dw, dbias, M, K, N, stream);
}
extern "C" int64_t tcct_pw_bwd_bn_supported(int K, int N, int post, int red_post, int split) {
    PwBwdMode md;
    md.split = split != 0; md.bnp = post; md.redp = red_post;
    return post >= 0 && pw_bwd_find(K, N, md) != nullptr;
}
static int pw_bwd_bn_impl(const void* x, const void* x2, const void* dz, PwBnBwd bn, int post, const float* w, const void* res, void* dx, void* dx2,
                          float* dw, float* dbias, int64_t M, int K, int N, int red_post, tcct_stream_t stream) {
    PwBwdMode md;
    md.split = x2 != nullptr; md.bnp = post; md.redp = red_post;
    TCCT_CHECK(tcct_pw_bwd_bn_supported(K, N, post, red_post, md.split ? 1 : 0), "pw_bwd_bn: K=%d N=%d post=%d red_post=%d split=%d unsupported", K, N, post,
               red_post, (int)md.split);
    TCCT_CHECK(bn.y != nullptr && (red_post < 0 || (bn.yprev && bn.abprev && bn.sums_prev)), "pw_bwd_bn: NULL argument");
    TCCT_CHECK(!md.split || (dx2 != nullptr && res == nullptr), "pw_bwd_bn: the concatenated form takes x2 / dx2 and no residual");
    return pw_bwd_impl(x, dz, w, md.split ? x2 : res, dx, md.split ? dx2 : nullptr, dw, dbias, M, K, N, stream, md, bn);
}
extern "C" int tcct_pw_bwd_bn(const void* x, const void* x2, const void* dz, const void* y, const float* coef, int post, const float* w,
                              const void* res, void* dx, void* dx2, float* dw, float* dbias, int64_t M, int K, int N, const void* y_prev,
                              const float* ab_prev, int red_post, double* sums_prev, tcct_stream_t stream) {
    TCCT_CHECK(coef != nullptr, "pw_bwd_bn: coef is NULL");
    return pw_bwd_bn_impl(x, x2, dz, pw_bn_coef(y, coef, y_prev, ab_prev, sums_prev), post, w, res, dx, dx2, dw, dbias, M, K, N, red_post, stream);
}
extern "C" int tcct_pw_bwd_bn_sums(const void* x, const void* x2, const void* dz, const void* y, const double* sums, int raw, const float* mean_rstd,
                                   const float* ab, float* dgamma, float* dbeta, int post, const float* w, const void* res, void* dx, void* dx2,
                                   float* dw, float* dbias, int64_t M, int K, int N, const void* y_prev, const float* ab_prev, int red_post,
                                   double* sums_prev, tcct_stream_t stream) {
    TCCT_CHECK(sums && mean_rstd && ab && dgamma && dbeta, "pw_bwd_bn_sums: NULL argument");
    return pw_bwd_bn_impl(x, x2, dz, pw_bn_sums(y, sums, raw, mean_rstd, ab, dgamma, dbeta, y_prev, ab_prev, sums_prev), post, w, res, dx, dx2, dw, dbias, M, K, N,
                          red_post, stream);
}
extern "C" int tcct_pw_bwd_bn_sums_xaff(const void* y_prev, const float* ab_prev, const void* dz, const void* y, const double* sums, int raw,
                                        const float* mean_rstd, const float* ab, float* dgamma, float* dbeta, const float* w, const void* res, void* dx,
                                        float* dw, float* dbias, int64_t M, int K, int N, int red_post, double* sums_prev, tcct_stream_t stream) {
    TCCT_CHECK(y_prev && ab_prev && sums && mean_rstd && ab && dgamma && dbeta && (red_post < 0 || sums_prev), "pw_bwd_bn_sums_xaff: NULL argument");
    PwBwdMode md;
    md.bnp = TCCT_ACT_NONE; md.redp = red_post; md.xap = TCCT_ACT_HSWISH;
    return pw_bwd_impl(y_prev, dz, w, res, dx, nullptr, dw, dbias, M, K, N, stream, md, pw_bn_sums(y, sums, raw, mean_rstd, ab, dgamma, dbeta, y_prev, ab_prev, sums_prev));
}
extern "C" int tcct_pw_bwd_gelu(const void* x1, const void* dy, const float* w, void* dx1, float* dw, float* dbias, int64_t M, int K, int N,
                                tcct_stream_t stream) {
    PwBwdMode md;
    md.gelu_x = true;
    return pw_bwd_impl(x1, dy, w, nullptr, dx1, nullptr, dw, dbias, M, K, N, stream, md);
}
extern "C" int tcct_pw_bwd_residual2_sum(const void* x, const void* dy_a, const void* dy_b, const float* w, const void* res, void* dx_sum, void* dx_plain, float* dw,
                                         float* dbias, int64_t M, int K, int N, tcct_stream_t stream) {
    TCCT_CHECK(dy_b != nullptr && res != nullptr && dx_plain != nullptr && dx_plain != dx_sum, "pw_bwd_residual2_sum: needs dy_b, res and two distinct outputs");
    PwBwdMode md;
    md.dy2 = true;
    return pw_bwd_impl(x, dy_a, w, res, dx_sum, dx_plain, dw, dbias, M, K, N, stream, md, pw_bn_dy2(dy_b));
}
extern "C" int tcct_pw_bwd_lnb(const void* x, const void* dy, const float* w, const void* t, const float* mean_rstd, const float* gamma, const void* res,
                               void* dt, float* dw, float* dbias, float* dgamma, float* dbeta, int64_t M, int K, int N, tcct_stream_t stream) {
    TCCT_CHECK(t && mean_rstd && gamma && res && dgamma && dbeta, "pw_bwd_lnb: NULL argument");
    PwBwdMode md;
    md.lnb = true;
    return pw_bwd_impl(x, dy, w, res, dt, nullptr, dw, dbias, M, K, N, stream, md, pw_bn_ln_front(t, gamma, mean_rstd, dgamma, dbeta));
}

template <int NT, int KT, bool STATS, bool SPLIT, bool RES = false, bool GX = false, int XAP = -1, bool AFF = false>
__global__ void __launch_bounds__(PWB, 2)
k_pw_fwd2(const bf16* __restrict__ x, const bf16* __restrict__ x2, const float* __restrict__ w, const float* __restrict__ bias,
          bf16* __restrict__ y, int64_t M, double* __restrict__ stats, int stat_pre, PwRes pr) {
    constexpr int K = 32 * KT, N = 32 * NT;
    constexpr int SX = 2 * K + 16, SW = 2 * K + 16;
    constexpr int XS = K / 16;
    extern __shared__ __attribute__((aligned(16))) unsigned char smem[];
    unsigned char* sX = smem;
    unsigned char* sW = sX + PB_P * SX;
    float* sB = reinterpret_cast<float*>(sW + N * SW);
    unsigned char* sS = reinterpret_cast<unsigned char*>(sB + N);
    const int tid = threadIdx.x, lane = tid & 63, wave = tid >> 6;
    const int r = lane & 31, hh = lane >> 5;
    for (int i = tid; i < N * (K / 8); i += PWB) {
        const int n = i / (K / 8), c8 = i - n * (K / 8);
        const float4 a = *reinterpret_cast<const float4*>(w + (int64_t)n * K + c8 * 8);
        const float4 b = *reinterpret_cast<const float4*>(w + (int64_t)n * K + c8 * 8 + 4);
        uint4 o;
        o.x = pack_bf16x2(a.x, a.y); o.y = pack_bf16x2(a.z, a.w); o.z = pack_bf16x2(b.x, b.y); o.w = pack_bf16x2(b.z, b.w);
        *reinterpret_cast<uint4*>(sW + n * SW + c8 * 16) = o;
    }
    if (tid < N) sB[tid] = bias ? bias[tid] : 0.f;
    float* sXA = reinterpret_cast<float*>(sS + 4 * 2560);
    if (XAP >= 0) for (int i = tid; i < 2 * K; i += PWB) sXA[i] = pr.xab[i];
    float* sAF = sXA + (XAP >= 0 ? 2 * K : 0);
    if (AFF) for (int i = tid; i < 2 * N; i += PWB) sAF[i] = pr.aff ? pr.aff[i] : (i < N ? 1.f : 0.f);
    float ss[STATS ? NT : 1][8], sq[STATS ? NT : 1][8];
#pragma unroll
    for (int a = 0; a < (STATS ? NT : 1); ++a)
#pragma unroll
        for (int k = 0; k < 8; ++k) ss[a][k] = sq[a][k] = 0.f;
    const int64_t tiles = (M + PB_P - 1) / PB_P;
    constexpr int KS = SPLIT ? K / 2 : K;
    const uint32_t xbytes = (uint32_t)(M * KS * 2), ybytes = (uint32_t)(M * N * 2);
    const __amdgpu_buffer_rsrc_t rx = __builtin_amdgcn_make_buffer_rsrc((void*)x, 0, xbytes, 0x00020000);
    const __amdgpu_buffer_rsrc_t rx2 = __builtin_amdgcn_make_buffer_rsrc((void*)(SPLIT ? x2 : x), 0, xbytes, 0x00020000);
    const __amdgpu_buffer_rsrc_t ro = __builtin_amdgcn_make_buffer_rsrc((void*)y, 0, ybytes, 0x00020000);
    const __amdgpu_buffer_rsrc_t rres = __builtin_amdgcn_make_buffer_rsrc((void*)(RES ? (const void*)pr.res : (const void*)y), 0, ybytes, 0x00020000);
    const __amdgpu_buffer_rsrc_t rpl = __builtin_amdgcn_make_buffer_rsrc((void*)((RES && pr.yplain) ? pr.yplain : y), 0, ybytes, 0x00020000);
    u32x4 px[XS];
    auto prefetch = [&](int64_t tile) {
        const uint32_t bx = (uint32_t)(tile * PB_P * KS * 2);
#pragma unroll
        for (int j = 0; j < XS; ++j) {
            if (SPLIT && j >= XS / 2) px[j] = __builtin_amdgcn_raw_buffer_load_b128(rx2, bx + (uint32_t)(tid + (j - XS / 2) * PWB) * 16u, 0, 0);
            else px[j] = __builtin_amdgcn_raw_buffer_load_b128(rx, bx + (uint32_t)(tid + j * PWB) * 16u, 0, 0);
        }
    };
    auto stage = [&]() {
#pragma unroll
        for (int j = 0; j < XS; ++j) {
            const int jj = (SPLIT && j >= XS / 2) ? j - XS / 2 : j;
            const int q = tid + jj * PWB, p = q / (KS / 8), c = q - p * (KS / 8);
            u32x4 xv_ = GX ? gelu8(px[j]) : px[j];
            if (XAP >= 0) xv_ = affine8<XAP < 0 ? 0 : XAP>(xv_, sXA + c * 8, sXA + K + c * 8);
            *reinterpret_cast<u32x4*>(sX + p * SX + ((SPLIT && j >= XS / 2) ? KS * 2 : 0) + c * 16) = xv_;
        }
    };
    const unsigned char* bB = sX + (32 * wave + r) * SX + hh * 16;
    int64_t tile = blockIdx.x;
    if (tile < tiles) {
        prefetch(tile);
        __syncthreads();
        stage();
        prefetch(tile + gridDim.x);
    }
    __syncthreads();
    for (; tile < tiles; tile += gridDim.x) {
        f32x16 acc[NT];
#pragma unroll
        for (int nt = 0; nt < NT; ++nt)
#pragma unroll
            for (int k = 0; k < 16; ++k) acc[nt][k] = 0.f;
#pragma unroll
        for (int st = 0; st < 2 * KT; ++st) {
            const bf16x8 fb = *reinterpret_cast<const bf16x8*>(bB + st * 32);
#pragma unroll
            for (int nt = 0; nt < NT; ++nt) {
                const bf16x8 fa = *reinterpret_cast<const bf16x8*>(sW + (nt * 32 + r) * SW + st * 32 + hh * 16);
                acc[nt] = __builtin_amdgcn_mfma_f32_32x32x16_bf16(fa, fb, acc[nt], 0, 0, 0);
// ... 359 lines not shown
```

tcct_amd/nets/tcct.py:

```python
import math

import torch
from torch import nn

from .. import ops
from .._lib import TcctError

KSIZES = (13, 11, 9, 7, 5)


def _conv(m, x, out_dtype=None, stats_pre=None):
    return ops.conv2d(x, m.weight, m.bias, stride=m.stride[0], pad=tuple(m.padding), out_dtype=out_dtype, stats_pre=stats_pre)


def _dw(m, x, add_input=False, bn_stats=False, deferred=None):
    return ops.dwconv3x3(x, m.weight, m.bias, stride=m.stride[0], add_input=add_input, bn_stats=bn_stats, deferred=deferred)


def _bn(m, x, pre=None, post=None, residual=None):
    return ops.batchnorm(x, m.weight, m.bias, m.running_mean, m.running_var, m.num_batches_tracked, eps=m.eps,
                         momentum=m.momentum, pre_act=pre, post_act=post, training=m.training, residual=residual)


def _bn_args(m):
# ... 206 lines not shown
        for k, split in window.items():
            self.conv_list.append(nn.Conv2d(split * Ch, split * Ch, (k, k), padding=(k // 2, k // 2), groups=split * Ch))
            self.head_splits.append(split)
        self.channel_splits = [x * Ch for x in self.head_splits]


class FactorAtt_ConvRelPosEnc(nn.Module):

    def __init__(self, dim, num_heads=8, qkv_bias=False, qk_scale=None, shared_crpe=None):
        super().__init__()
        self.num_heads = num_heads
        self.scale = qk_scale or (dim // num_heads) ** -0.5
        self.qkv = nn.Linear(dim, dim * 3, bias=qkv_bias)
        self.proj = nn.Linear(dim, dim)
        self.crpe = shared_crpe

    def mix(self, x, size):
        if sum(self.crpe.channel_splits) != x.shape[-1]:
            raise ValueError(f'crpe head splits {self.crpe.head_splits} do not cover {self.num_heads} heads')
        qkv = ops.conv2d(x, self.qkv.weight, self.qkv.bias)
        return ops.factor_att(qkv, size, self.num_heads, self.scale, self.crpe.conv_list)

    def forward(self, x, size):
        return ops.conv2d(self.mix(x, size), self.proj.weight, self.proj.bias)


class HydraAttention(nn.Module):

    def __init__(self, dim, num_heads=8, qkv_bias=False, qk_scale=None, shared_crpe=None):
        super().__init__()
        self.num_heads = num_heads
        self.scale = qk_scale or (dim // num_heads) ** -0.5
        self.qkv = nn.Linear(dim, dim * 3, bias=qkv_bias)
        self.proj = nn.Linear(dim, dim)
        self.crpe = shared_crpe

    def mix(self, x, size):
        if sum(self.crpe.channel_splits) != x.shape[-1]:
            raise ValueError(f'crpe head splits {self.crpe.head_splits} do not cover {self.num_heads} heads')
        qkv = ops.conv2d(x, self.qkv.weight, self.qkv.bias)
        return ops.hydra_att(qkv, size, self.num_heads, self.scale, self.crpe.conv_list)

    def forward(self, x, size):
        return ops.conv2d(self.mix(x, size), self.proj.weight, self.proj.bias)


class Mlp(nn.Module):

    def __init__(self, dim, hidden):
        super().__init__()
        self.fc1 = nn.Linear(dim, hidden)
        self.fc2 = nn.Linear(hidden, dim)


class MHCABlock(nn.Module):

    def __init__(self, dim, mlp_ratio, drop_path, shared_cpe, shared_crpe, att='pool', num_heads=8):
        super().__init__()
        self.cpe = shared_cpe
        self.crpe = shared_crpe
        if att == 'factor':
            self.att = FactorAtt_ConvRelPosEnc(dim, num_heads=num_heads, qkv_bias=True, shared_crpe=shared_crpe)
        elif att == 'hydra':
            self.att = HydraAttention(dim, num_heads=num_heads, qkv_bias=True, shared_crpe=shared_crpe)
        elif att != 'pool':
            raise ValueError(f"att must be 'pool' (MetaPool, tcct.py:449), 'factor' or 'hydra', got {att!r}")
        self.mlp = Mlp(dim, dim * mlp_ratio)
        self.drop_prob = float(drop_path)
        self.norm1 = nn.LayerNorm(dim, eps=1e-6)
        self.norm2 = nn.LayerNorm(dim, eps=1e-6)

    def forward(self, x, scales, fork=False):
        B, H, W, C = x.shape
        m = self.cpe.proj
        if fork:
            x, x_alias = ops.dwconv3x3_fork(x, m.weight, m.bias, stride=m.stride[0], add_input=True)
        else:
            x = _dw(m, x, add_input=True)
        t = x.view(B, H * W, C)
        s1, s2 = scales if scales is not None else (None, None)
        att = getattr(self, 'att', None)
        cur2 = None
        if att is None and ops.ln_metapool_residual_ok(t, self.norm1.weight, self.norm1.bias):
            if ops.LN_POOL_LN2:
                t, cur2, mr2 = ops.ln_metapool_residual_ln(t, self.norm1.weight, self.norm1.bias, self.norm1.eps, s1, self.norm2.weight, self.norm2.bias,
                                                           self.norm2.eps)
                m_ = self.mlp
                if ops.mlp_tail_ok(t, cur2, m_.fc1.weight, m_.fc1.bias, m_.fc2.weight, m_.fc2.bias):
                    t = ops.mlp_tail(t, cur2, mr2, self.norm2.weight, self.norm2.bias, m_.fc1.weight, m_.fc1.bias, m_.fc2.weight, m_.fc2.bias, s2)
                    return (t.view(B, H, W, C), x_alias) if fork else t.view(B, H, W, C)
            else:
                t = ops.ln_metapool_residual(t, self.norm1.weight, self.norm1.bias, self.norm1.eps, s1)
        else:
            cur, t = ops.layernorm_fork(t, self.norm1.weight, self.norm1.bias, self.norm1.eps)
            if att is not None:
                t = ops.linear_residual(att.mix(cur, (H, W)), att.proj.weight, att.proj.bias, t, s1)
            else:
                t = ops.metapool_residual(cur, t, s1)
        if cur2 is None:
            cur, t = ops.layernorm_fork(t, self.norm2.weight, self.norm2.bias, self.norm2.eps)
        else:
            cur = cur2
        if self.training or torch.is_grad_enabled() or not ops.INFER_FUSE:
            y1 = ops.conv2d(cur, self.mlp.fc1.weight, self.mlp.fc1.bias)
            if ops.gelu_linear_residual_ok(y1, self.mlp.fc2.weight, self.mlp.fc2.bias, t):
                t = ops.gelu_linear_residual(y1, self.mlp.fc2.weight, self.mlp.fc2.bias, t, s2)
                return (t.view(B, H, W, C), x_alias) if fork else t.view(B, H, W, C)
            h = ops.act(y1, 'gelu')
        else:
            h = ops.conv_bn_act(cur, self.mlp.fc1.weight, self.mlp.fc1.bias, post_act='gelu')
        t = ops.linear_residual(h, self.mlp.fc2.weight, self.mlp.fc2.bias, t, s2)
        return (t.view(B, H, W, C), x_alias) if fork else t.view(B, H, W, C)


class MHCAEncoder(nn.Module):

    def __init__(self, dim, num_heads, mlp_ratio, drop_path, att='pool'):
        super().__init__()
        self.cpe = ConvPosEnc(dim, k=3)
        self.crpe = ConvRelPosEnc(Ch=dim // num_heads, h=num_heads, window={3: 2, 5: 3, 7: 3})
        self.MHCA_layers = nn.ModuleList([MHCABlock(dim, mlp_ratio, drop_path, self.cpe, self.crpe, att=att, num_heads=num_heads)])

    def forward(self, x, scales, fork=False):
        return self.MHCA_layers[0](x, scales, fork)


class ResBlock(nn.Module):

    def __init__(self, dim):
        super().__init__()
        self.conv1 = Conv2d_BN(dim, dim, act=True)
        self.dwconv = nn.Conv2d(dim, dim, 3, 1, 1, bias=False, groups=dim)
        self.norm = nn.BatchNorm2d(dim)
        self.conv2 = Conv2d_BN(dim, dim)
        for m in (self.conv1.conv, self.dwconv, self.conv2.conv):
            fan_out = m.kernel_size[0] * m.kernel_size[1] * m.out_channels // m.groups
            m.weight.data.normal_(0, math.sqrt(2.0 / fan_out))

    def forward(self, x):
        return self.tail(self.conv1(x), x)

    def tail(self, f, x, flink=None):
        y = _dw(self.dwconv, f, bn_stats=self.norm.training, deferred=flink)
        c2, m = self.conv2, self.norm
        if (ops.batchnorm_deferred_ok(y, m.training, 'hswish') and c2.bn.training and not c2.act
                and ops.pw_conv_bn_ok(y, c2.conv.weight, None, True, None, None)):
            ya, link = ops.batchnorm_deferred(y, m.weight, m.bias, m.running_mean, m.running_var, m.num_batches_tracked, m.eps, m.momentum, 'hswish')
            return ops.pw_conv_bn(ya, c2.conv.weight, None, _bn_args(c2.bn), None, residual=x, deferred=link)
        if not m.training and not c2.bn.training and not c2.act and ops.invres_tail_eval_ok(y, c2.conv.weight, c2.conv.bias, x):
            mb = c2.bn
            return ops.invres_tail_eval(y, (m.weight, m.bias, m.running_mean, m.running_var, m.eps), c2.conv.weight, c2.conv.bias,
                                        (mb.weight, mb.bias, mb.running_mean, mb.running_var, mb.eps), x)
        f = _bn(self.norm, y, post='hswish')
        return self.conv2(f, residual=x, x_final=True)


class MHCA_stage(nn.Module):

    def __init__(self, embed_dim, out_embed_dim, num_heads, mlp_ratio, drop_path, att='pool'):
        super().__init__()
        self.mhca_blks = nn.ModuleList([MHCAEncoder(embed_dim, num_heads, mlp_ratio, drop_path, att=att)])
        self.InvRes = ResBlock(embed_dim)
        self.aggregate = Conv2d_BN(embed_dim * 2, out_embed_dim, act=True)

    def forward(self, x, scales):
        if torch.is_grad_enabled() and x.requires_grad:
            c1 = self.InvRes.conv1
            flink = None
            if ops.pw_conv_bn_ok(x, c1.conv.weight, None, c1.bn.training, None, 'hswish'):
                if ops.BN_DEFER_DW and x.shape[-1] % 4 == 0 and x.shape[-1] <= 256:
# ... 377 lines not shown
```

tcct_amd/ops.py:

```python
import os
import weakref

import torch

from ._lib import lib, dtype_code, TcctError, launch_on, F32, BF16

ACT = {None: 0, 'none': 0, 'lrelu': 1, 'hswish': 2, 'gelu': 3, 'sigmoid': 4, 'abs': 5}


class _ZeroPool:

    def __init__(self):
        self.buf = None
        self.off = 0
        self.active = False
        self.frozen = False

    def begin(self, device, nbytes=8 << 20):
        if self.buf is None or self.buf.device != device or self.buf.numel() < nbytes:
            if self.frozen:
                raise TcctError('the zero pool cannot be re-allocated after a training step was captured into a hipGraph '
                                f'(pool on {self.buf.device}, step on {device})')
            self.buf = torch.empty(nbytes, device=device, dtype=torch.uint8)
        self.buf.zero_()
# ... 941 lines not shown
class _GeluLinearResidual(_FastFunction):

    @staticmethod
    def forward(ctx, x1, w, bias, res, scale):
        _chk(x1, w, bias, res, scale)
        B, Nt, K = x1.shape
        Cout = w.shape[0]
        y = torch.empty((B, Nt, Cout), device=x1.device, dtype=x1.dtype)
        lib.pw_fwd_gelu_residual(x1, w, bias, res, scale, Nt, y, B * Nt, K, Cout)
        ctx.save_for_backward(x1, w)
        ctx.scale, ctx.params = scale, (w, bias)
        return y

    @staticmethod
    def backward(ctx, dy):
        x1, w = ctx.saved_tensors
        wsrc, bsrc = ctx.params
        dy = _c(dy)
        B, Nt, K = x1.shape
        Cout, M = w.shape[0], B * Nt
        dz = dy
        if ctx.scale is not None:
            dz = torch.empty_like(dy)
            lib.scale_rows(dy, ctx.scale, dz, B, dy.numel() // B, dtype_code(dy.dtype))
        dx1 = torch.empty_like(x1)
        dw = _grad_out(wsrc, tuple(w.shape))
        db = _grad_out(bsrc)
        lib.pw_bwd_gelu(x1, dz, w, dx1, dw, db, M, K, Cout)
        return dx1, _ret(dw, wsrc), _ret(db, bsrc), dy, None


class _MlpTail(_FastFunction):

    @staticmethod
    def forward(ctx, t1, cur2, mr2, g2, b2, w1, bias1, w2, bias2, scale):
        _chk(t1, cur2, mr2, g2, b2, w1, bias1, w2, bias2, scale)
        B, Nt, K = t1.shape
        M = B * Nt
        y1 = torch.empty_like(t1)
        lib.pw_fwd(cur2, w1, bias1, y1, M, K, K, 0, dtype_code(t1.dtype))
        t2 = torch.empty_like(t1)
        lib.pw_fwd_gelu_residual(y1, w2, bias2, t1, scale, Nt, t2, M, K, K)
        ctx.save_for_backward(t1, cur2, mr2, y1, g2, w1, w2)
        ctx.scale = scale
        ctx.params = (g2, b2, w1, bias1, w2, bias2)
        return t2

    @staticmethod
    def backward(ctx, dt2):
        t1, cur2, mr2, y1, g2, w1, w2 = ctx.saved_tensors
        g2p, b2p, w1p, bias1p, w2p, bias2p = ctx.params
        dt2 = _as(dt2, t1.dtype)
        B, Nt, K = t1.shape
        M = B * Nt
        dz = dt2
        if ctx.scale is not None:
            dz = torch.empty_like(dt2)
            lib.scale_rows(dt2, ctx.scale, dz, B, dt2.numel() // B, dtype_code(dt2.dtype))
        w1s = w1p if hasattr(w1p, '_grad_slot') or w1p._base is None else w1p._base
        w2s = w2p if hasattr(w2p, '_grad_slot') or w2p._base is None else w2p._base
        dy1 = torch.empty_like(y1)
        dw2, db2 = _grad_out(w2s, tuple(w2.shape)), _grad_out(bias2p)
        lib.pw_bwd_gelu(y1, dz, w2, dy1, dw2, db2, M, K, K)
        dt1 = torch.empty_like(t1)
        dw1, db1 = _grad_out(w1s, tuple(w1.shape)), _grad_out(bias1p)
        dg2, dbeta2 = _grad_out(g2p), _grad_out(b2p)
        lib.pw_bwd_lnb(cur2, dy1, w1, t1, mr2, g2, dt2, dt1, dw1, db1, dg2, dbeta2, M, K, K)
        return (dt1, None, None, _ret(dg2, g2p), _ret(dbeta2, b2p), _ret(dw1, w1s), _ret(db1, bias1p), _ret(dw2, w2s), _ret(db2, bias2p), None)


MLP_TAIL_FUSE = True


def mlp_tail_ok(t1, cur2, w1, bias1, w2, bias2):
    return (MLP_TAIL_FUSE and MLP_GELU_FUSE and FUSED_PW_BWD and torch.is_grad_enabled() and t1.dtype == torch.bfloat16 and t1.dim() == 3 and t1.shape[-1] == 64
            and cur2.shape == t1.shape and tuple(w1.shape) == (64, 64) and tuple(w2.shape) == (64, 64) and bias1 is not None and bias2 is not None
            and t1.is_contiguous() and cur2.is_contiguous() and t1.numel() * 2 < 2 ** 31)


def mlp_tail(t1, cur2, mr2, g2, b2, w1, bias1, w2, bias2, scale=None):
    return _MlpTail.apply(t1, cur2, mr2, g2, b2, w1, bias1, w2, bias2, scale)


def gelu_linear_residual_ok(x1, w, bias, res):
    return (MLP_GELU_FUSE and FUSED_PW_BWD and torch.is_grad_enabled() and x1.dtype == torch.bfloat16 and x1.dim() == 3 and w.dim() == 2
            and x1.shape[-1] in (64, 96) and w.shape[0] == x1.shape[-1] and w.shape[1] == x1.shape[-1] and bias is not None
            and res.shape == x1.shape and x1.numel() * 2 < 2 ** 31)


def gelu_linear_residual(x1, w, bias, res, scale=None):
    return _GeluLinearResidual.apply(x1, w, bias, res, scale)


class _Conv1x1AndSum(_FastFunction):

    @staticmethod
    def forward(ctx, x, w, bias, res):
        ctx.set_materialize_grads(False)
        _chk(x, w, bias, res)
        N_, H, W_, K = x.shape
        Cout = w.shape[0]
        d = torch.empty((N_, H, W_, Cout), device=x.device, dtype=x.dtype)
        s_ = torch.empty_like(d)
        lib.pw_fwd_residual(x, w, bias, res, None, 1, s_, d, N_ * H * W_, K, Cout)
        ctx.save_for_backward(x, w)
        ctx.params = (w, bias)
        return d, s_

    @staticmethod
    def backward(ctx, gd, gs):
        x, w = ctx.saved_tensors
        wsrc, bsrc = ctx.params
        if gd is None and gs is None:
            return None, None, None, None
        if gd is None or gs is None:
            dz = _c(gd if gs is None else gs)
        else:
            dz = torch.empty_like(gs)
            lib.add(_c(gd), _c(gs), dz, dz.numel(), dtype_code(dz.dtype))
        N_, H, W_, K = x.shape
        Cout, M = w.shape[0], N_ * H * W_
        dx = torch.empty_like(x)
        if FUSED_PW_BWD and _pw_bwd_ok(x, dz, K, K, Cout, 1, 1, 1, 0, 0):
            dw = _grad_out(wsrc, tuple(w.shape))
            db = _grad_out(bsrc)
            lib.pw_bwd(x, dz, w, None, dx, dw, db, M, K, Cout)
            return dx, _ret(dw, wsrc), _ret(db, bsrc), (None if gs is None else _c(gs))
        lib.pw_fwd(dz, w, None, dx, M, Cout, K, 1, dtype_code(x.dtype))
        with _wgrad_stream(_slot_written(wsrc, bsrc), x, dz):
            dw = _grad_out(wsrc, tuple(w.shape))
            db = _grad_out(bsrc)
            lib.pw_wgrad(x, dz, dw, db, M, K, Cout)
        return dx, _ret(dw, wsrc), _ret(db, bsrc), (None if gs is None else _c(gs))


class _UpSkipConv(_FastFunction):

    @staticmethod
    def forward(ctx, y, skip, w, bias, align, want_plain=True):
        ctx.set_materialize_grads(False)
        _chk(y, skip, w, bias)
        N_, H, W_, C = y.shape
        _, Ho, Wo, _ = skip.shape
        Cout = w.shape[0]
        u = torch.empty_like(skip)
        lib.bilinear_add_fwd(y, skip, u, N_, H, W_, C, Ho, Wo, int(align), dtype_code(y.dtype))
        s_ = torch.empty((N_, Ho, Wo, Cout), device=y.device, dtype=y.dtype)
        d = torch.empty_like(s_) if want_plain else None
        lib.pw_fwd_residual(u, w, bias, skip, None, 1, s_, d, N_ * Ho * Wo, C, Cout)
        ctx.save_for_backward(u, w)
        ctx.params = (w, bias)
        ctx.cfg = (N_, H, W_, C, Ho, Wo, int(align))
        if d is None:
            d = s_.new_empty(0)
            ctx.mark_non_differentiable(d)
        return d, s_

    @staticmethod
    def backward(ctx, gd, gs):
        u, w = ctx.saved_tensors
        wsrc, bsrc = ctx.params
        N_, H, W_, C, Ho, Wo, align = ctx.cfg
        if gd is None and gs is None:
            return None, None, None, None, None, None
        Cout, M = w.shape[0], N_ * Ho * Wo
        if (gd is not None and gs is not None and DY2_FUSE and FUSED_PW_BWD and C == 32 and Cout == 32 and u.dtype == torch.bfloat16
# ... 1200 lines not shown
        _chk(cur, t, scale)
        B, N, C = cur.shape
        y = torch.empty_like(cur)
        lib.metapool_residual_fwd(cur, t, scale, y, B, N, C, dtype_code(cur.dtype))
        ctx.scale = scale
        return y

    @staticmethod
    def backward(ctx, dy):
        dy = _c(dy)
        B, N, C = dy.shape
        dcur = torch.empty_like(dy)
        lib.metapool_scaled_bwd(dy, ctx.scale, dcur, B, N, C, dtype_code(dy.dtype))
        return dcur, dy, None


def metapool_residual(cur, t, scale=None):
    return _MetaPoolResidual.apply(cur, t, scale)


class _LnMetaPoolResidual(_FastFunction):

    @staticmethod
    def forward(ctx, t, gamma, beta, eps, scale):
        _chk(t, gamma, beta, scale)
        B, N, C = t.shape
        y = torch.empty_like(t)
        lib.ln_metapool_residual_fwd(t, y, B, N, C, gamma, beta, eps, scale, dtype_code(t.dtype))
        ctx.save_for_backward(t, gamma)
        ctx.beta_param, ctx.scale, ctx.eps = beta, scale, eps
        return y

    @staticmethod
    def backward(ctx, dy):
        t, gamma = ctx.saved_tensors
        dy = _as(dy, t.dtype)
        B, N, C = t.shape
        dt = torch.empty_like(t)
        dg, db = _grad_out(gamma), _grad_out(ctx.beta_param)
        lib.ln_metapool_residual_bwd(t, dy, dt, B, N, C, gamma, ctx.eps, ctx.scale, dg, db, dtype_code(t.dtype))
        return dt, _ret(dg, gamma), _ret(db, ctx.beta_param), None, None


class _LnMetaPoolResidualLn(_FastFunction):

    @staticmethod
    def forward(ctx, t, g1, b1, eps1, scale, g2, b2, eps2):
        ctx.set_materialize_grads(False)
        _chk(t, g1, b1, scale, g2, b2)
        B, N, C = t.shape
        y, y2 = torch.empty_like(t), torch.empty_like(t)
        mr2 = torch.empty(2 * B * N, device=t.device, dtype=torch.float32)
        lib.ln_metapool_residual_ln_fwd(t, y, y2, B, N, C, g1, b1, eps1, scale, g2, b2, eps2, mr2, dtype_code(t.dtype))
        ctx.save_for_backward(t, y, g1, g2, mr2)
        ctx.beta = (b1, b2)
        ctx.cfg = (eps1, scale)
        ctx.mark_non_differentiable(mr2)
        return y, y2, mr2

    @staticmethod
    def backward(ctx, dres, dcur, _dmr=None):
        t, y, g1, g2, mr2 = ctx.saved_tensors
        b1, b2 = ctx.beta
        eps1, scale = ctx.cfg
        B, N, C = t.shape
        dc = dtype_code(t.dtype)
        dg2 = db2 = None
        if dcur is not None:
            dcur = _as(dcur, t.dtype)
            dt1 = torch.empty_like(t)
            dg2, db2 = _grad_out(g2), _grad_out(b2)
            if dres is None:
                lib.layernorm_bwd(y, dcur, dt1, B * N, C, g2, mr2, dg2, db2, dc)
            else:
                lib.layernorm_bwd_add(y, dcur, _as(dres, t.dtype), dt1, B * N, C, g2, mr2, dg2, db2, dc)
        else:
            dt1 = _as(dres, t.dtype)
        dt = torch.empty_like(t)
        dg1, db1 = _grad_out(g1), _grad_out(b1)
        lib.ln_metapool_residual_bwd(t, dt1, dt, B, N, C, g1, eps1, scale, dg1, db1, dc)
        return dt, _ret(dg1, g1), _ret(db1, b1), None, None, _ret(dg2, g2), _ret(db2, b2), None


LN_POOL_FUSE = True


def ln_metapool_residual_ok(t, gamma, beta):
    return (LN_POOL_FUSE and t.dim() == 3 and t.is_cuda and t.is_contiguous() and t.dtype in (torch.float32, torch.bfloat16) and t.shape[-1] % 8 == 0
            and 16 <= t.shape[-1] <= 192 and t.shape[0] <= 65535 and t.shape[1] < 2 ** 30 and gamma is not None and beta is not None)


def ln_metapool_residual(t, gamma, beta, eps=1e-6, scale=None):
    return _LnMetaPoolResidual.apply(t, gamma, beta, float(eps), scale)


LN_POOL_LN2 = True


def ln_metapool_residual_ln(t, g1, b1, eps1, scale, g2, b2, eps2):
    return _LnMetaPoolResidualLn.apply(t, g1, b1, float(eps1), scale, g2, b2, float(eps2))


def metapool(x):
    return _MetaPool.apply(x)


class _FactorAtt(_FastFunction):

    @staticmethod
    def forward(ctx, qkv, H, W, heads, scale, *wb):
        _chk(qkv, *wb)
        B, N, C3 = qkv.shape
        C = C3 // 3
        if C * 3 != C3 or H * W != N or C % heads or (C // heads) % 4:
            raise TcctError(f'factor_att: qkv {tuple(qkv.shape)} does not fit size ({H},{W}) / heads {heads} (Ch must be a multiple of 4)')
        if sum(w.shape[0] for w in wb[0::2]) != C:
            raise TcctError('factor_att: the crpe window splits do not add up to the channel count')
        Ch, dt, dev = C // heads, dtype_code(qkv.dtype), qkv.device
        ws = torch.empty(lib.fatt_kstats_workspace_bytes(B, N, C), device=dev, dtype=torch.uint8)
        stats = torch.empty((B, C, 2), device=dev, dtype=torch.float32)
        lib.fatt_kstats(qkv, ws, stats, B, N, C, heads, dt)
        M = ZERO.get((B, heads, Ch, Ch), torch.float32, dev)
        lib.fatt_ktv(qkv, stats, M, B, N, C, heads, dt)
        cv = torch.empty((B, N, C), device=dev, dtype=qkv.dtype)
        off = 0
        for w, b in zip(wb[0::2], wb[1::2]):
            Cg, K = w.shape[0], w.shape[2]
            lib.dwk_strided_fwd(qkv[0, 0, 2 * C + off:], 3 * C, w, b, cv[0, 0, off:], C, B, H, W, Cg, K, 0, 0, dt)
            off += Cg
        out = torch.empty((B, N, C), device=dev, dtype=qkv.dtype)
        lib.fatt_apply_fwd(qkv, M, cv, out, float(scale), B, N, C, heads, dt)
        ctx.save_for_backward(qkv, stats, M, cv, *wb[0::2])
        ctx.cfg = (H, W, heads, float(scale))
        ctx.params = wb
        return out

    @staticmethod
    def backward(ctx, dout):
        qkv, stats, M, cv, *ws = ctx.saved_tensors
        H, W, heads, scale = ctx.cfg
        wb = ctx.params
        B, N, C3 = qkv.shape
        C = C3 // 3
        dt, dev = dtype_code(qkv.dtype), qkv.device
        dout = _as(dout, qkv.dtype)
        dM = ZERO.get(tuple(M.shape), torch.float32, dev)
        lib.fatt_dktv(qkv, dout, dM, scale, B, N, C, heads, dt)
        dqkv = torch.empty_like(qkv)
        dcv = torch.empty_like(cv)
        lib.fatt_apply_bwd(qkv, stats, M, dM, cv, dout, dqkv, dcv, scale, B, N, C, heads, dt)
        grads, off = [], 0
        for w, b in zip(wb[0::2], wb[1::2]):
            Cg, K = w.shape[0], w.shape[2]
            lib.dwk_strided_fwd(dcv[0, 0, off:], C, w, None, dqkv[0, 0, 2 * C + off:], 3 * C, B, H, W, Cg, K, 1, 1, dt)
            dw = _grad_out(w)
            db = _grad_out(b) if b is not None else None
            lib.dwk_strided_wgrad(qkv[0, 0, 2 * C + off:], 3 * C, dcv[0, 0, off:], C, dw, db, B, H, W, Cg, K, dt)
            grads += [_ret(dw, w), _ret(db, b)]
            off += Cg
        return (dqkv, None, None, None, None) + tuple(grads)


def factor_att(qkv, size, heads, scale, crpe_convs):
    wb = []
    for m in crpe_convs:
        wb += [m.weight, m.bias]
    return _FactorAtt.apply(qkv, int(size[0]), int(size[1]), int(heads), float(scale), *wb)


class _HydraAtt(_FastFunction):

    @staticmethod
    def forward(ctx, qkv, H, W, heads, scale, *wb):
        _chk(qkv, *wb)
        B, N, C3 = qkv.shape
        C = C3 // 3
        if C * 3 != C3 or H * W != N or C % heads or (C // heads) % 4:
            raise TcctError(f'hydra_att: qkv {tuple(qkv.shape)} does not fit size ({H},{W}) / heads {heads} (Ch must be a multiple of 4)')
        if sum(w.shape[0] for w in wb[0::2]) != C:
            raise TcctError('hydra_att: the crpe window splits do not add up to the channel count')
        dt, dev = dtype_code(qkv.dtype), qkv.device
        ws = torch.empty(lib.hydra_kv_workspace_bytes(B, N, C), device=dev, dtype=torch.uint8)
        kv = torch.empty((B, C), device=dev, dtype=torch.float32)
# ... 905 lines not shown
```

Before: 415.0 B-scans/s.

## Fuse LayerNorm, MLP fc1/GELU/fc2 and residual into one forward kernel

Adds a persistent MFMA kernel for 64-channel MLP blocks. Per tile it applies the second LayerNorm from precomputed row stats, runs fc1, stores the pre-GELU activation, applies GELU, runs fc2 and adds the scaled residual, all through LDS. The preceding LN/metapool kernel gains a stats-only mode, so the normalized tensor no longer has to be written. Backward recomputes the LN output inside a new pw_bwd_lnx variant instead of reading it. This cuts HBM traffic and kernel launches, at the cost of more kernel complexity and recomputation in backward.

```diff
diff --git a/include/tcct_hip.h b/include/tcct_hip.h
--- a/include/tcct_hip.h
+++ b/include/tcct_hip.h
@@ -191,7 +191,12 @@
                               float* dbias, int64_t M, int K, int N, tcct_stream_t stream);
 int tcct_pw_bwd_lnb(const void* x, const void* dy, const float* w, const void* t, const float* mean_rstd, const float* gamma, const void* res, void* dt,
                     float* dw, float* dbias, float* dgamma, float* dbeta, int64_t M, int K, int N, tcct_stream_t stream);
+int tcct_pw_bwd_lnx(const void* dy, const float* w, const void* t, const float* mean_rstd, const float* gamma, const float* beta, const void* res, void* dt,
+                    float* dw, float* dbias, float* dgamma, float* dbeta, int64_t M, int K, int N, tcct_stream_t stream);
 int tcct_pw_bwd_gelu(const void* x1, const void* dy, const float* w, void* dx1, float* dw, float* dbias, int64_t M, int K, int N, tcct_stream_t stream);
+int tcct_mlp64_fwd(const void* t1, const float* mean_rstd, const float* gamma2, const float* beta2, const float* w1, const float* b1, const float* w2,
+                   const float* b2, const float* scale, int64_t per_sample, void* y1, void* t2, int64_t M, tcct_stream_t stream);
+int64_t tcct_mlp64_fwd_grid_cap(void);
 int tcct_pw_dgrad_residual(const void* dy, const float* w, const void* res, void* dx_sum, void* dx_plain, int64_t M, int Nout, int K,
                            tcct_stream_t stream);
 int tcct_pw_fwd_cat2(const void* x1, const void* x2, int K1, const float* w, const float* bias, void* y, int64_t M, int K, int N,
@@ -266,6 +271,8 @@
                                   int dtype, tcct_stream_t stream);
 int tcct_ln_metapool_residual_ln_fwd(const void* t, void* y, void* y2, int B, int64_t N, int C, const float* gamma, const float* beta, float eps,
                                      const float* scale, const float* gamma2, const float* beta2, float eps2, float* mean_rstd2, int dtype, tcct_stream_t stream);
+int tcct_ln_metapool_residual_stats2_fwd(const void* t, void* y, int B, int64_t N, int C, const float* gamma, const float* beta, float eps, const float* scale,
+                                         float eps2, float* mean_rstd2, int dtype, tcct_stream_t stream);
 int tcct_ln_metapool_residual_bwd(const void* t, const void* dy, void* dt, int B, int64_t N, int C, const float* gamma, float eps, const float* scale,
                                   float* dgamma, float* dbeta, int dtype, tcct_stream_t stream);
 int tcct_maxpool2_fwd(const void* x, void* y, int N, int H, int W, int C, int dtype, tcct_stream_t stream);
diff --git a/tcct_amd/__init__.py b/tcct_amd/__init__.py
--- a/tcct_amd/__init__.py
+++ b/tcct_amd/__init__.py
@@ -8,6 +8,7 @@
 TCCT_FUSED_CONV_BWD TCCT_FUSED_PW_BWD TCCT_FUSE_AUX TCCT_GRAPH_ERRMODE TCCT_GRAPH_SHARED_POOL TCCT_HEAD_COMPOSE TCCT_HEAD_UPADD TCCT_LN_POOL TCCT_LN_POOL_LN2
 TCCT_MLP_GELU TCCT_MLP_TAIL TCCT_NORMADD_BAND TCCT_PACK_ALL TCCT_PW_FWD2 TCCT_TAIL_AUX TCCT_TAIL_AUX_LOW TCCT_TAIL_COMPOSE TCCT_TRAN_FUSE TCCT_TRAN_RED2
 TCCT_WGRAD_FRESH_EVENT TCCT_WGRAD_GENERIC TCCT_WGRAD_LINE TCCT_WGRAD_RECORD_STREAM TCCT_WGRAD_STREAM'''.split())
+LIVE_ENV = frozenset('TCCT_WIDE_CONV TCCT_CONV_CHAIN TCCT_STREAMS TCCT_MLP_FWD_FUSE'.split())
 _set = sorted(v for v in RETIRED_ENV if v in _os.environ)
 if _set:
     _warnings.warn('tcct_amd: ' + ', '.join(_set) + ' no longer have any effect (retired environment switches; use the tcct_amd.ops module constants or '
diff --git a/tcct_amd/csrc/common.h b/tcct_amd/csrc/common.h
--- a/tcct_amd/csrc/common.h
+++ b/tcct_amd/csrc/common.h
@@ -183,6 +183,22 @@
 }
 
 typedef __attribute__((__vector_size__(4 * sizeof(unsigned int)))) unsigned int u32x4;
+typedef __attribute__((__vector_size__(2 * sizeof(unsigned int)))) unsigned int u32x2;
+__device__ __forceinline__ u32x4 ln_apply8(u32x4 v, float mean, float rstd, const float* __restrict__ gam, const float* __restrict__ bet) {
+    u32x4 o;
+#pragma unroll
+    for (int k = 0; k < 4; ++k)
+        o[k] = pack_bf16x2((__uint_as_float(v[k] << 16) - mean) * rstd * gam[2 * k] + bet[2 * k],
+                           (__uint_as_float(v[k] & 0xffff0000u) - mean) * rstd * gam[2 * k + 1] + bet[2 * k + 1]);
+    return o;
+}
+__device__ __forceinline__ u32x4 gelu8(u32x4 v) {
+    u32x4 o;
+#pragma unroll
+    for (int k = 0; k < 4; ++k)
+        o[k] = pack_bf16x2(act_c<TCCT_ACT_GELU>(__uint_as_float(v[k] << 16)), act_c<TCCT_ACT_GELU>(__uint_as_float(v[k] & 0xffff0000u)));
+    return o;
+}
 __device__ __forceinline__ void lds_dma16(const u32x4& rsrc, uint32_t voff, uint32_t lds_addr) {
     unsigned keep;
     asm volatile("s_nop 4\n\ts_mov_b32 %0, m0\n\ts_mov_b32 m0, %3\n\ts_nop 0\n\tbuffer_load_dwordx4 %1, %2, 0 offen lds\n\ts_mov_b32 m0, %0"
diff --git a/tcct_amd/csrc/ln_pool.hip b/tcct_amd/csrc/ln_pool.hip
--- a/tcct_amd/csrc/ln_pool.hip
+++ b/tcct_amd/csrc/ln_pool.hip
@@ -70,7 +70,7 @@
     rstd = rsqrtf(q * invC + eps);
 }
 
-template <typename T, int LP, bool LN2>
+template <typename T, int LP, int LN2>
 __global__ void __launch_bounds__(LP_T)
 k_ln_metapool_fwd(const T* __restrict__ t, T* __restrict__ y, int N, int C, const float* __restrict__ gamma, const float* __restrict__ beta, float eps,
                   const float* __restrict__ scale, T* __restrict__ y2, const float* __restrict__ gamma2, const float* __restrict__ beta2, float eps2,
@@ -89,7 +89,7 @@
     }
     float gam2[8], bet2[8];
 #pragma unroll
-    for (int k = 0; k < 8; ++k) { gam2[k] = (LN2 && act) ? gamma2[c0 + k] : 0.f; bet2[k] = (LN2 && act) ? beta2[c0 + k] : 0.f; }
+    for (int k = 0; k < 8; ++k) { gam2[k] = (LN2 == 1 && act) ? gamma2[c0 + k] : 0.f; bet2[k] = (LN2 == 1 && act) ? beta2[c0 + k] : 0.f; }
     const int64_t img = (int64_t)blockIdx.y * N;
     const T* tb = t + img * C + c0;
     T* yb = y + img * C + c0;
@@ -137,10 +137,12 @@
                     float mean2, rstd2;
                     row_stats<LP>(orr, act, invC, eps2, mean2, rstd2);
                     if (gl == 0) { mean_rstd2[2 * (img + n)] = mean2; mean_rstd2[2 * (img + n) + 1] = rstd2; }
-                    f8 b;
-#pragma unroll
-                    for (int k = 0; k < 8; ++k) b.v[k] = (orr.v[k] - mean2) * rstd2 * gam2[k] + bet2[k];
-                    if (act) st8(y2 + (img + n) * C + c0, b);
+                    if (LN2 == 1) {
+                        f8 b;
+#pragma unroll
+                        for (int k = 0; k < 8; ++k) b.v[k] = (orr.v[k] - mean2) * rstd2 * gam2[k] + bet2[k];
+                        if (act) st8(y2 + (img + n) * C + c0, b);
+                    }
                 }
             }
             prev = cur; cur = nxt; ccur = cnxt; e = xn;
@@ -250,8 +252,9 @@
     const int64_t strips = (N + LNP_STRIP - 1) / LNP_STRIP;
 #define LNPF(LP_, L2) hipLaunchKernelGGL((k_ln_metapool_fwd<T, LP_, L2>), dim3((unsigned)((strips + LP_T / LP_ - 1) / (LP_T / LP_)), (unsigned)B), dim3(LP_T), 0, \
                                          (hipStream_t)stream, (const T*)t, (T*)y, (int)N, C, gamma, beta, eps, scale, (T*)y2, gamma2, beta2, eps2, mean_rstd2)
-    if (y2) { TCCT_DISPATCH(dtype, if (C <= 64) LNPF(8, true); else if (C <= 128) LNPF(16, true); else LNPF(32, true)); }
-    else { TCCT_DISPATCH(dtype, if (C <= 64) LNPF(8, false); else if (C <= 128) LNPF(16, false); else LNPF(32, false)); }
+    if (y2) { TCCT_DISPATCH(dtype, if (C <= 64) LNPF(8, 1); else if (C <= 128) LNPF(16, 1); else LNPF(32, 1)); }
+    else if (mean_rstd2) { TCCT_DISPATCH(dtype, if (C <= 64) LNPF(8, 2); else if (C <= 128) LNPF(16, 2); else LNPF(32, 2)); }
+    else { TCCT_DISPATCH(dtype, if (C <= 64) LNPF(8, 0); else if (C <= 128) LNPF(16, 0); else LNPF(32, 0)); }
 #undef LNPF
     TCCT_LAUNCH_OK();
 }
@@ -264,6 +267,11 @@
                                                 tcct_stream_t stream) {
     TCCT_CHECK(y2 && gamma2 && beta2 && mean_rstd2, "ln_metapool_residual_ln_fwd: NULL argument");
     return ln_metapool_fwd_impl(t, y, B, N, C, gamma, beta, eps, scale, y2, gamma2, beta2, eps2, mean_rstd2, dtype, stream);
+}
+extern "C" int tcct_ln_metapool_residual_stats2_fwd(const void* t, void* y, int B, int64_t N, int C, const float* gamma, const float* beta, float eps,
+                                                    const float* scale, float eps2, float* mean_rstd2, int dtype, tcct_stream_t stream) {
+    TCCT_CHECK(mean_rstd2, "ln_metapool_residual_stats2_fwd: NULL argument");
+    return ln_metapool_fwd_impl(t, y, B, N, C, gamma, beta, eps, scale, nullptr, nullptr, nullptr, eps2, mean_rstd2, dtype, stream);
 }
 extern "C" int tcct_ln_metapool_residual_bwd(const void* t, const void* dy, void* dt, int B, int64_t N, int C, const float* gamma, float eps, const float* scale,
                                              float* dgamma, float* dbeta, int dtype, tcct_stream_t stream) {
diff --git a/tcct_amd/csrc/mlp_fwd.hip b/tcct_amd/csrc/mlp_fwd.hip
--- /dev/null
+++ b/tcct_amd/csrc/mlp_fwd.hip
@@ -0,0 +1,155 @@
+#include "common.h"
+
+typedef __attribute__((ext_vector_type(8))) __bf16 bf16x8;
+typedef __attribute__((ext_vector_type(16))) float f32x16;
+
+#define MLP_T 256
+#define MLP_P 128
+#define MLP_C 64
+#define MLP_SX (2 * MLP_C + 16)
+#define MLP_GRID_CAP 512
+
+__global__ void __launch_bounds__(MLP_T, 2)
+k_mlp64_fwd(const bf16* __restrict__ t1, const float* __restrict__ mean_rstd, const float* __restrict__ gamma, const float* __restrict__ beta,
+            const float* __restrict__ w1, const float* __restrict__ b1, const float* __restrict__ w2, const float* __restrict__ b2,
+            const float* __restrict__ scale, uint32_t per_sample, uint32_t samples, bf16* __restrict__ y1, bf16* __restrict__ t2, int64_t M) {
+    constexpr int C = MLP_C, SX = MLP_SX;
+    extern __shared__ __attribute__((aligned(16))) unsigned char smem[];
+    unsigned char* sX = smem;
+    unsigned char* sW1 = sX + MLP_P * SX;
+    unsigned char* sW2 = sW1 + C * SX;
+    float* sB = reinterpret_cast<float*>(sW2 + C * SX);
+    const int tid = threadIdx.x, lane = tid & 63, wave = tid >> 6;
+    const int r = lane & 31, hh = lane >> 5;
+    const int rl = lane >> 3, ch = lane & 7;
+    for (int i = tid; i < 2 * C * (C / 8); i += MLP_T) {
+        const int m = i / (C * (C / 8)), n = (i / (C / 8)) % C, c8 = i % (C / 8);
+        const float* w = m ? w2 : w1;
+        const float4 a = *reinterpret_cast<const float4*>(w + n * C + c8 * 8);
+        const float4 b = *reinterpret_cast<const float4*>(w + n * C + c8 * 8 + 4);
+        uint4 o;
+        o.x = pack_bf16x2(a.x, a.y); o.y = pack_bf16x2(a.z, a.w); o.z = pack_bf16x2(b.x, b.y); o.w = pack_bf16x2(b.z, b.w);
+        *reinterpret_cast<uint4*>((m ? sW2 : sW1) + n * SX + c8 * 16) = o;
+    }
+    if (tid < C) { sB[tid] = b1[tid]; sB[C + tid] = b2[tid]; }
+    float gam[8], bet[8];
+#pragma unroll
+    for (int k = 0; k < 8; ++k) { gam[k] = gamma[ch * 8 + k]; bet[k] = beta[ch * 8 + k]; }
+    const int64_t tiles = (M + MLP_P - 1) / MLP_P;
+    const uint32_t abytes = (uint32_t)(M * C * 2);
+    const bool has_scale = scale != nullptr;
+    const __amdgpu_buffer_rsrc_t rt = __builtin_amdgcn_make_buffer_rsrc((void*)t1, 0, abytes, 0x00020000);
+    const __amdgpu_buffer_rsrc_t ry = __builtin_amdgcn_make_buffer_rsrc((void*)y1, 0, abytes, 0x00020000);
+    const __amdgpu_buffer_rsrc_t ro = __builtin_amdgcn_make_buffer_rsrc((void*)t2, 0, abytes, 0x00020000);
+    const __amdgpu_buffer_rsrc_t rm = __builtin_amdgcn_make_buffer_rsrc((void*)mean_rstd, 0, (uint32_t)(M * 8), 0x00020000);
+    const __amdgpu_buffer_rsrc_t rs = __builtin_amdgcn_make_buffer_rsrc((void*)(has_scale ? scale : mean_rstd), 0, has_scale ? samples * 4u : 0u, 0x00020000);
+    unsigned char* wrow = sX + 32 * wave * SX;
+    unsigned char* prow = wrow + rl * SX + ch * 16;
+    const unsigned char* bB = wrow + r * SX + hh * 16;
+    const uint32_t lane_off = (uint32_t)(wave * 4096 + lane * 16);
+    const uint32_t lane_row = (uint32_t)(32 * wave + rl);
+    struct Set { u32x4 x[4]; u32x2 m[4]; float s[4]; };
+    auto prefetch = [&](Set& p, int64_t tile) {
+        const uint32_t bx = (uint32_t)tile * (uint32_t)(MLP_P * C * 2) + lane_off, row0 = (uint32_t)tile * MLP_P + lane_row;
+#pragma unroll
+        for (int s = 0; s < 4; ++s) p.x[s] = __builtin_amdgcn_raw_buffer_load_b128(rt, bx + 1024u * s, 0, 0);
+#pragma unroll
+        for (int s = 0; s < 4; ++s) p.m[s] = __builtin_amdgcn_raw_buffer_load_b64(rm, (row0 + 8u * s) * 8u, 0, 0);
+#pragma unroll
+        for (int s = 0; s < 4; ++s) p.s[s] = __uint_as_float(__builtin_amdgcn_raw_buffer_load_b32(rs, ((row0 + 8u * s) / per_sample) * 4u, 0, 0));
+    };
+    auto stage = [&](const Set& p) {
+#pragma unroll
+        for (int s = 0; s < 4; ++s) {
+            *reinterpret_cast<u32x4*>(prow + 8 * s * SX) = ln_apply8(p.x[s], __uint_as_float(p.m[s][0]), __uint_as_float(p.m[s][1]), gam, bet);
+        }
+    };
+    auto gemm = [&](const unsigned char* sW, f32x16 (&acc)[2]) {
+#pragma unroll
+        for (int nt = 0; nt < 2; ++nt)
+#pragma unroll
+            for (int k = 0; k < 16; ++k) acc[nt][k] = 0.f;
+#pragma unroll
+        for (int st = 0; st < 4; ++st) {
+            const bf16x8 fb = *reinterpret_cast<const bf16x8*>(bB + st * 32);
+#pragma unroll
+            for (int nt = 0; nt < 2; ++nt) {
+                const bf16x8 fa = *reinterpret_cast<const bf16x8*>(sW + (nt * 32 + r) * SX + st * 32 + hh * 16);
+                acc[nt] = __builtin_amdgcn_mfma_f32_32x32x16_bf16(fa, fb, acc[nt], 0, 0, 0);
+            }
+        }
+    };
+    auto to_rows = [&](const f32x16 (&acc)[2], const float* bias) {
+#pragma unroll
+        for (int nt = 0; nt < 2; ++nt)
+#pragma unroll
+            for (int q = 0; q < 4; ++q) {
+                const float4 bq = *reinterpret_cast<const float4*>(bias + nt * 32 + 8 * q + 4 * hh);
+                uint2 o;
+                o.x = pack_bf16x2(acc[nt][4 * q] + bq.x, acc[nt][4 * q + 1] + bq.y);
+                o.y = pack_bf16x2(acc[nt][4 * q + 2] + bq.z, acc[nt][4 * q + 3] + bq.w);
+                *reinterpret_cast<uint2*>(wrow + r * SX + (nt * 32 + 8 * q + 4 * hh) * 2) = o;
+            }
+    };
+    auto step = [&](Set& cur, const Set& nxt, int64_t tile) {
+        const uint32_t bo = (uint32_t)tile * (uint32_t)(MLP_P * C * 2) + lane_off;
+        f32x16 acc[2];
+        wave_lds_fence();
+        gemm(sW1, acc);
+        wave_lds_fence();
+        to_rows(acc, sB);
+        wave_lds_fence();
+#pragma unroll
+        for (int s = 0; s < 4; ++s) {
+            const u32x4 o = *reinterpret_cast<const u32x4*>(prow + 8 * s * SX);
+            __builtin_amdgcn_raw_buffer_store_b128(o, ry, bo + 1024u * s, 0, 0);
+            *reinterpret_cast<u32x4*>(prow + 8 * s * SX) = gelu8(o);
+        }
+        wave_lds_fence();
+        gemm(sW2, acc);
+        wave_lds_fence();
+        to_rows(acc, sB + C);
+        wave_lds_fence();
+#pragma unroll
+        for (int s = 0; s < 4; ++s) {
+            u32x4 o = *reinterpret_cast<const u32x4*>(prow + 8 * s * SX);
+            const u32x4 rv = cur.x[s];
+            const float sc_ = has_scale ? cur.s[s] : 1.f;
+#pragma unroll
+            for (int k = 0; k < 4; ++k)
+                o[k] = pack_bf16x2(__uint_as_float(rv[k] << 16) + sc_ * __uint_as_float(o[k] << 16),
+                                   __uint_as_float(rv[k] & 0xffff0000u) + sc_ * __uint_as_float(o[k] & 0xffff0000u));
+            __builtin_amdgcn_raw_buffer_store_b128(o, ro, bo + 1024u * s, 0, 0);
+        }
+        wave_lds_fence();
+        __builtin_amdgcn_sched_barrier(0);
+        prefetch(cur, tile + 2 * (int64_t)gridDim.x);
+        stage(nxt);
+    };
+    Set a, b;
+    int64_t tile = blockIdx.x;
+    prefetch(a, tile);
+    prefetch(b, tile + gridDim.x);
+    stage(a);
+    __syncthreads();
+    for (; tile < tiles; tile += 2 * (int64_t)gridDim.x) {
+        step(a, b, tile);
+        if (tile + (int64_t)gridDim.x >= tiles) break;
+        step(b, a, tile + gridDim.x);
+    }
+}
+
+extern "C" int64_t tcct_mlp64_fwd_grid_cap() { return MLP_GRID_CAP; }
+
+extern "C" int tcct_mlp64_fwd(const void* t1, const float* mean_rstd, const float* gamma2, const float* beta2, const float* w1, const float* b1, const float* w2,
+                              const float* b2, const float* scale, int64_t per_sample, void* y1, void* t2, int64_t M, tcct_stream_t stream) {
+    TCCT_CHECK(t1 && mean_rstd && gamma2 && beta2 && w1 && b1 && w2 && b2 && y1 && t2, "mlp64_fwd: NULL argument");
+    TCCT_CHECK(M > 0 && M * (int64_t)(MLP_C * 2) < (1LL << 31), "mlp64_fwd: M=%lld: tensor exceeds the 2 GiB buffer-descriptor range", (long long)M);
+    TCCT_CHECK(per_sample >= 1 && per_sample <= M, "mlp64_fwd: per_sample=%lld outside 1..M", (long long)per_sample);
+    const int64_t tiles = (M + MLP_P - 1) / MLP_P;
+    const size_t lds = (size_t)MLP_P * MLP_SX + 2 * (size_t)MLP_C * MLP_SX + 2 * MLP_C * sizeof(float);
+    const int64_t gx = tiles < MLP_GRID_CAP ? tiles : MLP_GRID_CAP;
+    tcct_launch<k_mlp64_fwd, 64 * 1024>(dim3((unsigned)gx), dim3(MLP_T), lds, (hipStream_t)stream, (const bf16*)t1, mean_rstd, gamma2, beta2, w1, b1, w2, b2, scale,
+                                        (uint32_t)per_sample, (uint32_t)((M + per_sample - 1) / per_sample), (bf16*)y1, (bf16*)t2, M);
+    TCCT_LAUNCH_OK();
+}
diff --git a/tcct_amd/csrc/pw_mfma.hip b/tcct_amd/csrc/pw_mfma.hip
--- a/tcct_amd/csrc/pw_mfma.hip
+++ b/tcct_amd/csrc/pw_mfma.hip
@@ -712,13 +712,6 @@
 
 #define PB_P 128
 
-__device__ __forceinline__ u32x4 gelu8(u32x4 v) {
-    u32x4 o;
-#pragma unroll
-    for (int k = 0; k < 4; ++k)
-        o[k] = pack_bf16x2(act_c<TCCT_ACT_GELU>(__uint_as_float(v[k] << 16)), act_c<TCCT_ACT_GELU>(__uint_as_float(v[k] & 0xffff0000u)));
-    return o;
-}
 __device__ __forceinline__ float gelu_grad1(float x) { float c, p; gauss_cdf_pdf(x, c, p); return c + x * p; }
 template <int KIND> __device__ __forceinline__ u32x4 affine8(u32x4 v, const float* __restrict__ a, const float* __restrict__ b) {
     const float4 a0 = *reinterpret_cast<const float4*>(a), a1 = *reinterpret_cast<const float4*>(a + 4);
@@ -737,7 +730,7 @@
     if (KIND == TCCT_ACT_HSWISH) return u < -3.f ? 0.f : (u <= 3.f ? (2.f * u + 3.f) * (1.f / 6.f) : 1.f);
     return 1.f;
 }
-template <int NT, int KT, bool SPLIT = false, int BNP = -1, int REDP = -1, bool GX = false, int XAP = -1, bool LNB = false, bool DY2 = false>
+template <int NT, int KT, bool SPLIT = false, int BNP = -1, int REDP = -1, bool GX = false, int XAP = -1, bool LNB = false, bool DY2 = false, bool LNX = false>
 __global__ void __launch_bounds__(PWB, 2)
 k_pw_bwd(const bf16* __restrict__ x, const bf16* __restrict__ dy, const float* __restrict__ w, const bf16* __restrict__ res,
          bf16* __restrict__ dx, bf16* __restrict__ dx_plain, float* __restrict__ dw, float* __restrict__ dbias, int64_t M, PwBnBwd bn) {
@@ -774,6 +767,7 @@
     }
     if (RED || XAP >= 0) for (int i = tid; i < 2 * (SPLIT ? K / 2 : K); i += PWB) sP[i] = bn.abprev[i];
     if (LNB) for (int i = tid; i < K; i += PWB) sP[i] = bn.abprev[i];
+    if (LNX) for (int i = tid; i < K; i += PWB) sP[K + i] = bn.ab[i];
     constexpr int RKT = LNB ? KT : (RED ? (SPLIT ? KT / 2 : KT) : 1);
     float rs[RKT][8], rq[RKT][8];
 #pragma unroll
@@ -798,7 +792,9 @@
     const __amdgpu_buffer_rsrc_t rp = __builtin_amdgcn_make_buffer_rsrc((void*)(dx_plain ? dx_plain : dx), 0, xbytes, 0x00020000);
     const __amdgpu_buffer_rsrc_t ry = __builtin_amdgcn_make_buffer_rsrc((void*)((BN || DY2) ? bn.y : dy), 0, dbytes, 0x00020000);
     const __amdgpu_buffer_rsrc_t ryp = __builtin_amdgcn_make_buffer_rsrc((void*)((RED || LNB) ? bn.yprev : x), 0, xbytes, 0x00020000);
+    const __amdgpu_buffer_rsrc_t rmr = __builtin_amdgcn_make_buffer_rsrc((void*)(LNX ? (const void*)bn.mean_rstd : (const void*)x), 0, LNX ? (uint32_t)(M * 8) : 0u, 0x00020000);
     u32x4 px[XS], pd[DS], py[(BN || DY2) ? DS : 1];
+    u32x2 pmr[LNX ? XS : 1];
     auto prefetch = [&](int64_t tile) {
         const uint32_t bx = (uint32_t)(tile * PB_P * KS * 2), bd = (uint32_t)(tile * PB_P * N * 2);
 #pragma unroll
@@ -811,12 +807,17 @@
         if (BN || DY2) {
 #pragma unroll
             for (int j = 0; j < DS; ++j) py[j] = __builtin_amdgcn_raw_buffer_load_b128(ry, bd + (uint32_t)(tid + j * PWB) * 16u, 0, 0);
+        }
+        if (LNX) {
+#pragma unroll
+            for (int j = 0; j < XS; ++j) pmr[j] = __builtin_amdgcn_raw_buffer_load_b64(rmr, ((uint32_t)tile * PB_P + (uint32_t)(tid + j * PWB) / (K / 8)) * 8u, 0, 0);
         }
     };
     auto stage_x1 = [&](int j, u32x4 xv_) {
         const int jj = (SPLIT && j >= XS / 2) ? j - XS / 2 : j;
         const int q = tid + jj * PWB, p = q / (KS / 8), c = q - p * (KS / 8);
         if (GX) xv_ = gelu8(xv_);
+        if (LNX) xv_ = ln_apply8(xv_, __uint_as_float(pmr[LNX ? j : 0][0]), __uint_as_float(pmr[LNX ? j : 0][1]), sP + c * 8, sP + K + c * 8);
         if (XAP >= 0) xv_ = affine8<XAP < 0 ? 0 : XAP>(xv_, sP + c * 8, sP + KS + c * 8);
         *reinterpret_cast<u32x4*>(sX + p * SX + ((SPLIT && j >= XS / 2) ? KS * 2 : 0) + c * 16) = xv_;
     };
@@ -1154,7 +1155,7 @@
     }
 }
 
-struct PwBwdMode { bool split = false; int bnp = -1, redp = -1; bool gelu_x = false; int xap = -1; bool lnb = false, dy2 = false; };
+struct PwBwdMode { bool split = false; int bnp = -1, redp = -1; bool gelu_x = false; int xap = -1; bool lnb = false, dy2 = false, lnx = false; };
 static PwBnBwd pw_bn_coef(const void* y, const float* coef, const void* y_prev, const float* ab_prev, double* sums_prev) {
     PwBnBwd b{};
     b.y = (const bf16*)y; b.coef = coef; b.yprev = (const bf16*)y_prev; b.abprev = ab_prev; b.sums_prev = sums_prev;
@@ -1166,9 +1167,9 @@
     b.sums = sums; b.raw = raw; b.mean_rstd = mean_rstd; b.ab = ab; b.dgamma = dgamma; b.dbeta = dbeta;
     return b;
 }
-static PwBnBwd pw_bn_ln_front(const void* t, const float* gamma, const float* mean_rstd, float* dgamma, float* dbeta) {
+static PwBnBwd pw_bn_ln_front(const void* t, const float* gamma, const float* mean_rstd, float* dgamma, float* dbeta, const float* beta = nullptr) {
     PwBnBwd b{};
-    b.yprev = (const bf16*)t; b.abprev = gamma; b.mean_rstd = mean_rstd; b.dgamma = dgamma; b.dbeta = dbeta;
+    b.yprev = (const bf16*)t; b.abprev = gamma; b.mean_rstd = mean_rstd; b.dgamma = dgamma; b.dbeta = dbeta; b.ab = beta;
     return b;
 }
 static PwBnBwd pw_bn_dy2(const void* dy_b) {
@@ -1178,9 +1179,10 @@
 }
 
 typedef void (*PwBwdLaunch)(dim3, dim3, size_t, hipStream_t, const bf16*, const bf16*, const float*, const bf16*, bf16*, bf16*, float*, float*, int64_t, PwBnBwd);
-struct PwBwdRow { int nt, kt; bool split; int bnp, redp; bool gx; int xap; bool lnb, dy2; PwBwdLaunch launch; };
+struct PwBwdRow { int nt, kt; bool split; int bnp, redp; bool gx; int xap; bool lnb, dy2, lnx; PwBwdLaunch launch; };
 static_assert(TCCT_ACT_HSWISH == 2 && TCCT_ACT_NONE == 0, "activation codes are template arguments below");
-#define PWB_ROW(NT, KT, SP, BN, RD, GX, XA, LN, D2) {NT, KT, SP, BN, RD, GX, XA, LN, D2, tcct_launch<k_pw_bwd<NT, KT, SP, BN, RD, GX, XA, LN, D2>, 160 * 1024>}
+#define PWB_ROWX(NT, KT, SP, BN, RD, GX, XA, LN, D2, LX) {NT, KT, SP, BN, RD, GX, XA, LN, D2, LX, tcct_launch<k_pw_bwd<NT, KT, SP, BN, RD, GX, XA, LN, D2, LX>, 160 * 1024>}
+#define PWB_ROW(NT, KT, SP, BN, RD, GX, XA, LN, D2) PWB_ROWX(NT, KT, SP, BN, RD, GX, XA, LN, D2, false)
 #define PWB_PLAIN(NT, KT, SP) PWB_ROW(NT, KT, SP, -1, -1, false, -1, false, false)
 #define PWB_BN(NT, KT, SP, BN, RD) PWB_ROW(NT, KT, SP, BN, RD, false, -1, false, false)
 static const PwBwdRow pw_bwd_table[] = {
@@ -1195,24 +1197,26 @@
     PWB_ROW(2, 2, false, 0, 2, false, 2, false, false), PWB_ROW(3, 3, false, 0, -1, false, 2, false, false),
     PWB_ROW(2, 2, false, -1, -1, true, -1, false, false), PWB_ROW(3, 3, false, -1, -1, true, -1, false, false),
     PWB_ROW(2, 2, false, -1, -1, false, -1, true, false),
+    PWB_ROWX(2, 2, false, -1, -1, false, -1, true, false, true),
     PWB_ROW(1, 1, false, -1, -1, false, -1, false, true),
 };
 #undef PWB_BN
 #undef PWB_PLAIN
 #undef PWB_ROW
+#undef PWB_ROWX
 static const PwBwdRow* pw_bwd_find(int K, int N, const PwBwdMode& md) {
     if (K % 32 || N % 32) return nullptr;
     for (const PwBwdRow& r : pw_bwd_table)
         if (r.nt == N / 32 && r.kt == K / 32 && r.split == md.split && r.bnp == md.bnp && r.redp == md.redp && r.gx == md.gelu_x && r.xap == md.xap && r.lnb == md.lnb &&
-            r.dy2 == md.dy2) return &r;
+            r.dy2 == md.dy2 && r.lnx == md.lnx) return &r;
     return nullptr;
 }
 
 static int pw_bwd_impl(const void* x, const void* dy, const float* w, const void* res, void* dx, void* dx_plain, float* dw, float* dbias,
                        int64_t M, int K, int N, tcct_stream_t stream, const PwBwdMode& md = PwBwdMode(), PwBnBwd bn = PwBnBwd{}) {
     const PwBwdRow* row = pw_bwd_find(K, N, md);
-    TCCT_CHECK(row != nullptr, "pw_bwd: K=%d N=%d unsupported: no kernel for NT=%d KT=%d SPLIT=%d BNP=%d REDP=%d GX=%d XAP=%d LNB=%d DY2=%d", K, N, N / 32, K / 32,
-               (int)md.split, md.bnp, md.redp, (int)md.gelu_x, md.xap, (int)md.lnb, (int)md.dy2);
+    TCCT_CHECK(row != nullptr, "pw_bwd: K=%d N=%d unsupported: no kernel for NT=%d KT=%d SPLIT=%d BNP=%d REDP=%d GX=%d XAP=%d LNB=%d DY2=%d LNX=%d", K, N, N / 32, K / 32,
+               (int)md.split, md.bnp, md.redp, (int)md.gelu_x, md.xap, (int)md.lnb, (int)md.dy2, (int)md.lnx);
     TCCT_CHECK(M > 0 && M * (int64_t)(K > N ? K : N) * 2 < (1LL << 31), "pw_bwd: tensor exceeds the 2 GiB buffer-descriptor range");
     const int NT = N / 32, KT = K / 32;
     const int SX = 64 * KT + ((KT & 1) ? 0 : 64), SD = 64 * NT + ((NT & 1) ? 0 : 64), SW = 2 * N + 16;
@@ -1312,6 +1316,13 @@
     PwBwdMode md;
     md.lnb = true;
     return pw_bwd_impl(x, dy, w, res, dt, nullptr, dw, dbias, M, K, N, stream, md, pw_bn_ln_front(t, gamma, mean_rstd, dgamma, dbeta));
+}
+extern "C" int tcct_pw_bwd_lnx(const void* dy, const float* w, const void* t, const float* mean_rstd, const float* gamma, const float* beta, const void* res,
+                               void* dt, float* dw, float* dbias, float* dgamma, float* dbeta, int64_t M, int K, int N, tcct_stream_t stream) {
+    TCCT_CHECK(t && mean_rstd && gamma && beta && res && dgamma && dbeta, "pw_bwd_lnx: NULL argument");
+    PwBwdMode md;
+    md.lnb = md.lnx = true;
+    return pw_bwd_impl(t, dy, w, res, dt, nullptr, dw, dbias, M, K, N, stream, md, pw_bn_ln_front(t, gamma, mean_rstd, dgamma, dbeta, beta));
 }
 
 template <int NT, int KT, bool STATS, bool SPLIT, bool RES = false, bool GX = false, int XAP = -1, bool AFF = false>
diff --git a/tcct_amd/nets/tcct.py b/tcct_amd/nets/tcct.py
--- a/tcct_amd/nets/tcct.py
+++ b/tcct_amd/nets/tcct.py
@@ -312,10 +312,18 @@
         att = getattr(self, 'att', None)
         cur2 = None
         if att is None and ops.ln_metapool_residual_ok(t, self.norm1.weight, self.norm1.bias):
+            m_ = self.mlp
+            if ops.LN_POOL_LN2 and ops.mlp_block_ok(t, m_.fc1.weight, m_.fc1.bias, m_.fc2.weight, m_.fc2.bias):
+                if ops.MLP_BWD_LNX:
+                    t, mr2 = ops.ln_metapool_residual_stats2(t, self.norm1.weight, self.norm1.bias, self.norm1.eps, s1, self.norm2.eps)
+                else:
+                    t, cur2, mr2 = ops.ln_metapool_residual_ln(t, self.norm1.weight, self.norm1.bias, self.norm1.eps, s1, self.norm2.weight, self.norm2.bias,
+                                                               self.norm2.eps)
+                t = ops.mlp_block(t, mr2, self.norm2.weight, self.norm2.bias, m_.fc1.weight, m_.fc1.bias, m_.fc2.weight, m_.fc2.bias, s2, cur2)
+                return (t.view(B, H, W, C), x_alias) if fork else t.view(B, H, W, C)
             if ops.LN_POOL_LN2:
                 t, cur2, mr2 = ops.ln_metapool_residual_ln(t, self.norm1.weight, self.norm1.bias, self.norm1.eps, s1, self.norm2.weight, self.norm2.bias,
                                                            self.norm2.eps)
-                m_ = self.mlp
                 if ops.mlp_tail_ok(t, cur2, m_.fc1.weight, m_.fc1.bias, m_.fc2.weight, m_.fc2.bias):
                     t = ops.mlp_tail(t, cur2, mr2, self.norm2.weight, self.norm2.bias, m_.fc1.weight, m_.fc1.bias, m_.fc2.weight, m_.fc2.bias, s2)
                     return (t.view(B, H, W, C), x_alias) if fork else t.view(B, H, W, C)
diff --git a/tcct_amd/ops.py b/tcct_amd/ops.py
--- a/tcct_amd/ops.py
+++ b/tcct_amd/ops.py
@@ -1047,6 +1047,59 @@
     return _MlpTail.apply(t1, cur2, mr2, g2, b2, w1, bias1, w2, bias2, scale)
 
 
+class _MlpBlock(_FastFunction):
+
+    @staticmethod
+    def forward(ctx, t1, mr2, g2, b2, w1, bias1, w2, bias2, scale, cur2):
+        _chk(t1, mr2, g2, b2, w1, bias1, w2, bias2, scale, cur2)
+        B, Nt, K = t1.shape
+        y1, t2 = torch.empty_like(t1), torch.empty_like(t1)
+        lib.mlp64_fwd(t1, mr2, g2, b2, w1, bias1, w2, bias2, scale, Nt, y1, t2, B * Nt)
+        ctx.save_for_backward(t1, mr2, y1, g2, b2, w1, w2, cur2)
+        ctx.scale = scale
+        ctx.params = (g2, b2, w1, bias1, w2, bias2)
+        return t2
+
+    @staticmethod
+    def backward(ctx, dt2):
+        t1, mr2, y1, g2, b2, w1, w2, cur2 = ctx.saved_tensors
+        g2p, b2p, w1p, bias1p, w2p, bias2p = ctx.params
+        dt2 = _as(dt2, t1.dtype)
+        B, Nt, K = t1.shape
+        M = B * Nt
+        dz = dt2
+        if ctx.scale is not None:
+            dz = torch.empty_like(dt2)
+            lib.scale_rows(dt2, ctx.scale, dz, B, dt2.numel() // B, dtype_code(dt2.dtype))
+        w1s = w1p if hasattr(w1p, '_grad_slot') or w1p._base is None else w1p._base
+        w2s = w2p if hasattr(w2p, '_grad_slot') or w2p._base is None else w2p._base
+        dy1 = torch.empty_like(y1)
+        dw2, db2 = _grad_out(w2s, tuple(w2.shape)), _grad_out(bias2p)
+        lib.pw_bwd_gelu(y1, dz, w2, dy1, dw2, db2, M, K, K)
+        dt1 = torch.empty_like(t1)
+        dw1, db1 = _grad_out(w1s, tuple(w1.shape)), _grad_out(bias1p)
+        dg2, dbeta2 = _grad_out(g2p), _grad_out(b2p)
+        if cur2 is None:
+            lib.pw_bwd_lnx(dy1, w1, t1, mr2, g2, b2, dt2, dt1, dw1, db1, dg2, dbeta2, M, K, K)
+        else:
+            lib.pw_bwd_lnb(cur2, dy1, w1, t1, mr2, g2, dt2, dt1, dw1, db1, dg2, dbeta2, M, K, K)
+        return (dt1, None, _ret(dg2, g2p), _ret(dbeta2, b2p), _ret(dw1, w1s), _ret(db1, bias1p), _ret(dw2, w2s), _ret(db2, bias2p), None, None)
+
+
+MLP_FWD_FUSE = os.environ.get('TCCT_MLP_FWD_FUSE', '1') != '0'
+MLP_BWD_LNX = True
+
+
+def mlp_block_ok(t1, w1, bias1, w2, bias2):
+    return (MLP_FWD_FUSE and MLP_TAIL_FUSE and MLP_GELU_FUSE and FUSED_PW_BWD and torch.is_grad_enabled() and t1.dtype == torch.bfloat16 and t1.dim() == 3
+            and t1.shape[-1] == 64 and tuple(w1.shape) == (64, 64) and tuple(w2.shape) == (64, 64) and bias1 is not None and bias2 is not None
+            and t1.is_contiguous() and t1.numel() * 2 < 2 ** 31)
+
+
+def mlp_block(t1, mr2, g2, b2, w1, bias1, w2, bias2, scale=None, cur2=None):
+    return _MlpBlock.apply(t1, mr2, g2, b2, w1, bias1, w2, bias2, scale, cur2)
+
+
 def gelu_linear_residual_ok(x1, w, bias, res):
     return (MLP_GELU_FUSE and FUSED_PW_BWD and torch.is_grad_enabled() and x1.dtype == torch.bfloat16 and x1.dim() == 3 and w.dim() == 2
             and x1.shape[-1] in (64, 96) and w.shape[0] == x1.shape[-1] and w.shape[1] == x1.shape[-1] and bias is not None
@@ -2413,6 +2466,34 @@
         return dt, _ret(dg1, g1), _ret(db1, b1), None, None, _ret(dg2, g2), _ret(db2, b2), None
 
 
+class _LnMetaPoolResidualStats2(_FastFunction):
+
+    @staticmethod
+    def forward(ctx, t, g1, b1, eps1, scale, eps2):
+        ctx.set_materialize_grads(False)
+        _chk(t, g1, b1, scale)
+        B, N, C = t.shape
+        y = torch.empty_like(t)
+        mr2 = torch.empty(2 * B * N, device=t.device, dtype=torch.float32)
+        lib.ln_metapool_residual_stats2_fwd(t, y, B, N, C, g1, b1, eps1, scale, eps2, mr2, dtype_code(t.dtype))
+        ctx.save_for_backward(t, g1)
+        ctx.beta_param, ctx.scale, ctx.eps = b1, scale, eps1
+        ctx.mark_non_differentiable(mr2)
+        return y, mr2
+
+    @staticmethod
+    def backward(ctx, dy, _dmr=None):
+        if dy is None:
+            return None, None, None, None, None, None
+        t, g1 = ctx.saved_tensors
+        dy = _as(dy, t.dtype)
+        B, N, C = t.shape
+        dt = torch.empty_like(t)
+        dg, db = _grad_out(g1), _grad_out(ctx.beta_param)
+        lib.ln_metapool_residual_bwd(t, dy, dt, B, N, C, g1, ctx.eps, ctx.scale, dg, db, dtype_code(t.dtype))
+        return dt, _ret(dg, g1), _ret(db, ctx.beta_param), None, None, None
+
+
 LN_POOL_FUSE = True
 
 
@@ -2430,6 +2511,10 @@
 
 def ln_metapool_residual_ln(t, g1, b1, eps1, scale, g2, b2, eps2):
     return _LnMetaPoolResidualLn.apply(t, g1, b1, float(eps1), scale, g2, b2, float(eps2))
+
+
+def ln_metapool_residual_stats2(t, g1, b1, eps1, scale, eps2):
+    return _LnMetaPoolResidualStats2.apply(t, g1, b1, float(eps1), scale, float(eps2))
 
 
 def metapool(x):
```

Measured after the change: 418.4 B-scans/s (median of 6 runs). No clear change (+0.8%).
